# sen-ye/dmvae

Hardware: AMD Instinct MI355X
Metric: images/sec DMVAE train step @256x256 (higher is better)
Workload: dtype bf16

## Files before the change

### dmvae_amd/_lib.py

```python
from __future__ import annotations

import ctypes
import os
from ctypes import POINTER, Structure, c_char_p, c_double, c_float, c_int, c_int32, c_longlong, c_size_t, c_uint, c_ulonglong, c_void_p

_HERE = os.path.dirname(os.path.abspath(__file__))
LIB_PATH = os.environ.get("DMVAE_LIB") or os.path.join(_HERE, "libdmvae_hip.so")


class ConvDesc(Structure):
    _fields_ = [("n", c_int32), ("h", c_int32), ("w", c_int32), ("cin", c_int32), ("cout", c_int32),
                ("ks", c_int32), ("upsample", c_int32), ("act", c_int32), ("out_f32", c_int32), ("stride", c_int32), ("transposed", c_int32),
                ("w_layout", c_int32)]


class PackEntry(Structure):
    _fields_ = [("src", c_void_p), ("dst", c_void_p), ("dst2", c_void_p),
                ("cout", c_int32), ("cin", c_int32), ("T", c_int32), ("rows_pad", c_int32), ("cols_pad", c_int32), ("mode", c_int32), ("subpixel", c_int32),
                ("reserved", c_int32), ("start", c_ulonglong), ("count", c_ulonglong)]


class WtEntry(Structure):
    _fields_ = [("src", c_void_p), ("dst", c_void_p), ("N", c_int32), ("K", c_int32), ("start", c_uint), ("tiles_x", c_uint)]


class OdeTerms(Structure):
    _fields_ = [("k", c_void_p * 7), ("c", c_float * 7), ("nk", c_int32), ("k_bf16", c_int32)]


class ModelTerms(Structure):
    _fields_ = [("kind", c_int32), ("c0", c_float), ("dv", c_float), ("nsig", c_float)]


IMAGE_RECORD_WORDS = 12
IMAGE_OUT_U8_NHWC, IMAGE_OUT_F32_NCHW = 0, 1


ABI_VERSION = 9

SIGNATURES = {
    "dmvae_last_error": (c_char_p, []),
    "dmvae_abi_version": (c_int, []),
    "dmvae_rms_modulate_fwd_f32": (c_int, [c_void_p] * 6 + [c_size_t, c_int, c_int, c_int, c_float, c_void_p]),
    "dmvae_rms_modulate_bwd_f32": (c_int, [c_void_p] * 8 + [c_size_t, c_int, c_int, c_int, c_void_p]),
    "dmvae_layernorm_bwd_full_f32": (c_int, [c_void_p] * 5 + [c_size_t, c_int, c_float, c_void_p]),
    "dmvae_bcast_rows_f32": (c_int, [c_int] + [c_void_p] * 4 + [c_size_t, c_int, c_int, c_int, c_void_p]),
    "dmvae_colsum_groups_f32": (c_int, [c_void_p, c_void_p, c_int, c_int, c_int, c_int, c_void_p]),
    "dmvae_swiglu_fwd_f32": (c_int, [c_void_p, c_void_p, c_size_t, c_int, c_void_p]),
    "dmvae_swiglu_bwd_f32": (c_int, [c_void_p, c_void_p, c_void_p, c_size_t, c_int, c_void_p]),
    "dmvae_qknorm_rope_fwd_f32": (c_int, [c_void_p] * 9 + [c_int] * 5 + [c_float, c_void_p]),
    "dmvae_qknorm_rope_bwd_f32": (c_int, [c_void_p] * 12 + [c_int] * 5 + [c_void_p]),
    "dmvae_reparam_kl_workspace": (c_size_t, [c_size_t, c_int]),
    "dmvae_reparam_kl_fwd": (c_int, [c_void_p] * 5 + [c_size_t, c_size_t, c_int, c_int, c_void_p]),
    "dmvae_reparam_kl_bwd": (c_int, [c_void_p] * 4 + [c_float, c_void_p, c_size_t, c_int, c_int, c_void_p]),
    "dmvae_conv2d_nhwc_fwd": (c_int, [c_void_p, c_void_p, c_void_p, c_void_p, c_void_p, POINTER(ConvDesc), c_void_p]),
    "dmvae_conv2d_nhwc_fwd_gnstats_workspace": (c_size_t, [POINTER(ConvDesc), c_int]),
    "dmvae_conv2d_nhwc_fwd_gnstats": (c_int, [c_void_p] * 7 + [c_size_t, c_int, c_float, POINTER(ConvDesc), c_void_p]),
    "dmvae_conv2d_nhwc_wgrad_workspace": (c_size_t, [POINTER(ConvDesc)]),
    "dmvae_gemm_nt_batched": (c_int, [c_void_p] * 5 + [c_int] * 4 + [c_longlong] * 3 + [c_int, c_int, c_void_p]),
    "dmvae_gemm_tn_batched_workspace": (c_size_t, [c_int, c_int, c_int, c_int]),
    "dmvae_gemm_tn_batched": (c_int, [c_void_p] * 4 + [c_size_t] + [c_int] * 4 + [c_longlong] * 3 + [c_float, c_int, c_void_p]),
    "dmvae_set_dynamic": (c_int, [c_int]),
    "dmvae_linear_rows_supported": (c_int, [c_int, c_int, c_int]),
    "dmvae_linear_rows_bf16": (c_int, [c_void_p] * 4 + [c_int] * 10 + [c_void_p]),
    "dmvae_linear_rows_wgrad": (c_int, [c_void_p] * 4 + [c_int] * 6 + [c_void_p]),
    "dmvae_linear_bf16": (c_int, [c_void_p] * 4 + [c_int] * 10 + [c_void_p]),
    "dmvae_linear_bf16_swiglu_pre": (c_int, [c_void_p] * 5 + [c_int] * 9 + [c_void_p]),
    "dmvae_linear_bf16_sk_supported": (c_int, [c_int] * 5),
    "dmvae_linear_bf16_sk_workspace": (c_size_t, [c_int] * 5),
    "dmvae_linear_bf16_sk": (c_int, [c_void_p] * 5 + [c_size_t] + [c_int] * 11 + [c_void_p]),
    "dmvae_linear_bf16_batched_supported": (c_int, [c_int] * 4),
    "dmvae_linear_bf16_batched": (c_int, [c_void_p] * 3 + [c_int] * 7 + [c_longlong] * 3 + [c_int, c_void_p]),
    "dmvae_linear_bf16_plan": (c_int, [c_int, c_int, c_int, POINTER(c_int), POINTER(c_int)]),
    "dmvae_linear_weight_t_kmajor": (c_int, [c_void_p, c_void_p, c_int, c_int, c_void_p]),
    "dmvae_pack_entry_bytes": (c_size_t, []),
    "dmvae_pack_weights_batched": (c_int, [c_void_p, c_int, c_ulonglong, c_int, c_void_p]),
    "dmvae_softmax_rows_fwd": (c_int, [c_void_p, c_void_p, c_int, c_int, c_float, c_void_p]),
    "dmvae_softmax_rows_bwd": (c_int, [c_void_p, c_void_p, c_void_p, c_int, c_int, c_float, c_void_p]),
    "dmvae_transpose_bf16": (c_int, [c_void_p, c_void_p, c_int, c_int, c_int, c_void_p]),
    "dmvae_pack_conv_weight": (c_int, [c_void_p, c_void_p] + [c_int] * 6 + [c_void_p]),
    "dmvae_pack_conv_weight_v2": (c_int, [c_void_p, c_void_p, c_void_p] + [c_int] * 6 + [c_void_p]),
    "dmvae_conv_halo_applies": (c_int, [POINTER(ConvDesc)]),
    "dmvae_conv_kmajor_applies": (c_int, [POINTER(ConvDesc)]),
    "dmvae_subpixel_weight": (c_int, [c_void_p, c_void_p, c_int, c_int, c_void_p]),
    "dmvae_subpixel_weight_fold": (c_int, [c_void_p, c_void_p, c_int, c_int, c_int, c_void_p]),
    "dmvae_colsum_bf16": (c_int, [c_void_p, c_void_p, c_void_p, c_size_t, c_size_t, c_int, c_int, c_void_p]),
    "dmvae_conv_out_wgrad_workspace": (c_size_t, [c_int, c_int, c_int, c_int, c_int]),
    "dmvae_conv_out_wgrad": (c_int, [c_void_p, c_void_p, c_void_p, c_void_p, c_size_t, c_int, c_int, c_int, c_int, c_int, c_int, c_void_p]),
    "dmvae_sumpool2x2_nhwc": (c_int, [c_void_p, c_void_p, c_int, c_int, c_int, c_int, c_void_p]),
    "dmvae_maxpool2x2_nhwc": (c_int, [c_void_p, c_void_p, c_int, c_int, c_int, c_int, c_void_p]),
    "dmvae_maxpool2x2_relu_bwd_nhwc": (c_int, [c_void_p, c_void_p, c_void_p, c_void_p, c_int, c_int, c_int, c_int, c_void_p]),
    "dmvae_relu_bwd": (c_int, [c_void_p, c_void_p, c_void_p, c_size_t, c_void_p]),
    "dmvae_leaky_relu_bwd": (c_int, [c_void_p, c_void_p, c_void_p, c_size_t, c_float, c_void_p]),
    "dmvae_sde_euler_step": (c_int, [c_void_p, c_void_p, c_int, c_void_p, c_void_p, c_void_p, c_size_t] + [c_float] * 6 + [c_void_p]),
    "dmvae_image_to_u8": (c_int, [c_void_p, c_void_p, c_size_t, c_int, c_int, c_int, c_void_p]),
    "dmvae_ode_rk_combine": (c_int, [c_void_p, POINTER(OdeTerms), c_void_p, c_size_t, c_int, c_void_p]),
    "dmvae_ode_error_ratio_workspace": (c_size_t, [c_size_t]),
    "dmvae_ode_error_ratio": (c_int, [c_void_p, c_void_p, POINTER(OdeTerms), c_float, c_float, c_int, c_void_p, c_void_p, c_void_p, c_size_t, c_void_p]),
    "dmvae_ode_dense_output": (c_int, [c_void_p] * 5 + [c_int, c_float, c_float, c_void_p, c_size_t, c_void_p]),
    "dmvae_ode_hutchinson_pack": (c_int, [c_void_p, c_int, c_void_p, c_void_p, c_void_p, c_void_p, c_int, c_size_t, c_void_p]),
    "dmvae_cfg_combine": (c_int, [c_void_p, c_int, c_void_p, c_int, c_int, c_size_t, c_int, c_float, c_void_p, c_float, c_void_p]),
    "dmvae_sde_heun_perturb": (c_int, [c_void_p, c_void_p, c_void_p, c_size_t, c_float, c_float, c_void_p]),
    "dmvae_sde_heun_predict": (c_int, [c_void_p, c_void_p, c_int, c_void_p, c_void_p, c_size_t] + [c_float] * 4 + [c_void_p]),
    "dmvae_sde_heun_correct": (c_int, [c_void_p, c_void_p, c_void_p, c_void_p, c_int, c_void_p, c_size_t] + [c_float] * 4 + [c_void_p]),
    "dmvae_sde_last_step": (c_int, [c_void_p, c_void_p, c_int, c_void_p, c_size_t, c_int] + [c_float] * 5 + [c_void_p]),
    "dmvae_sde_euler_step_m": (c_int, [c_void_p, c_void_p, c_int, POINTER(ModelTerms), c_void_p, c_void_p, c_void_p, c_size_t] + [c_float] * 6 + [c_void_p]),
    "dmvae_sde_heun_predict_m": (c_int, [c_void_p, c_void_p, c_int, POINTER(ModelTerms), c_void_p, c_void_p, c_size_t] + [c_float] * 4 + [c_void_p]),
    "dmvae_sde_heun_correct_m": (c_int, [c_void_p, c_void_p, c_void_p, c_void_p, c_int, POINTER(ModelTerms), c_void_p, c_size_t] + [c_float] * 4 + [c_void_p]),
    "dmvae_sde_last_step_m": (c_int, [c_void_p, c_void_p, c_int, POINTER(ModelTerms), c_void_p, c_size_t, c_int] + [c_float] * 3 + [c_void_p]),
    "dmvae_model_velocity": (c_int, [c_void_p, c_void_p, c_int, POINTER(ModelTerms), c_void_p, c_size_t, c_void_p]),
    "dmvae_autoguidance_combine": (c_int, [c_void_p, c_int, c_void_p, c_int, c_int, c_void_p, c_int, c_size_t, c_int, c_float, c_void_p, c_float, c_float, c_void_p]),
    "dmvae_batchnorm_running_update": (c_int, [c_void_p, c_void_p, c_void_p, c_int, c_float, c_float, c_float, c_void_p]),
    "dmvae_diffaug_fwd": (c_int, [c_void_p] * 4 + [c_int] * 9 + [c_void_p]),
    "dmvae_diffaug_bwd": (c_int, [c_void_p] * 4 + [c_int] * 9 + [c_void_p]),
    "dmvae_im2col_nhwc_taps": (c_int, [c_void_p, c_void_p] + [c_int] * 8 + [c_void_p]),
    "dmvae_im2col_nhwc_sub": (c_int, [c_void_p, c_void_p] + [c_int] * 9 + [c_void_p]),
    "dmvae_col2im_nhwc": (c_int, [c_void_p, c_void_p] + [c_int] * 8 + [c_void_p]),
    "dmvae_nchw_f32_to_nhwc_bf16": (c_int, [c_void_p, c_void_p, c_int, c_int, c_int, c_int, c_void_p]),
    "dmvae_nhwc_to_nchw_f32": (c_int, [c_void_p, c_void_p, c_int, c_int, c_int, c_int, c_int, c_void_p]),
    "dmvae_silu_fwd": (c_int, [c_void_p, c_void_p, c_size_t, c_void_p]),
    "dmvae_silu_bwd": (c_int, [c_void_p, c_void_p, c_void_p, c_size_t, c_void_p]),
    "dmvae_layernorm_f32_bf16": (c_int, [c_void_p, c_void_p, c_void_p, c_void_p, c_int, c_int, c_float, c_void_p]),
    "dmvae_scale_residual_layernorm": (c_int, [c_void_p] * 6 + [c_int, c_int, c_float, c_void_p]),
    "dmvae_scale_residual_f32": (c_int, [c_void_p, c_void_p, c_void_p, c_size_t, c_int, c_void_p]),
    "dmvae_softmax_rows_bf16": (c_int, [c_void_p, c_void_p, c_size_t, c_int, c_float, c_void_p]),
    "dmvae_attention_qknorm_rope_bf16": (c_int, [c_void_p] * 6 + [c_int] * 4 + [c_float, c_float, c_void_p]),
    "dmvae_attention_qkv_lse_bf16": (c_int, [c_void_p] * 3 + [c_int] * 4 + [c_float, c_void_p]),
    "dmvae_attention_qkv_stream_bf16": (c_int, [c_void_p] * 3 + [c_int] * 4 + [c_float, c_void_p]),
    "dmvae_attention_heads_lse_bf16": (c_int, [c_void_p] * 5 + [c_int] * 5 + [c_float, c_void_p]),
    "dmvae_attention_heads_stream_bf16": (c_int, [c_void_p] * 5 + [c_int] * 5 + [c_float, c_void_p]),
    "dmvae_attention_wide_stream_bf16": (c_int, [c_void_p] * 5 + [c_int] * 3 + [c_float, c_void_p]),
    "dmvae_attention_wide_bwd_stream_bf16": (c_int, [c_void_p] * 10 + [c_int] * 3 + [c_float, c_void_p]),
    "dmvae_attention_bwd_heads_stream_bf16": (c_int, [c_void_p] * 10 + [c_int] * 5 + [c_float, c_void_p]),
    "dmvae_attention_bwd_qkv_lse_bf16": (c_int, [c_void_p] * 5 + [c_int] * 4 + [c_float, c_void_p]),
    "dmvae_attention_bwd_qkv_stream_bf16": (c_int, [c_void_p] * 6 + [c_int] * 4 + [c_float, c_void_p]),
    "dmvae_attention_bwd_heads_lse_bf16": (c_int, [c_void_p] * 9 + [c_int] * 5 + [c_float, c_void_p]),
    "dmvae_vit_bwd_workspace": (c_size_t, [c_int]),
    "dmvae_layernorm_bwd_f32": (c_int, [c_void_p] * 7 + [c_size_t, c_int, c_int, c_float, c_int, c_void_p]),
    "dmvae_layerscale_bwd": (c_int, [c_void_p] * 6 + [c_size_t, c_int, c_int, c_int, c_void_p]),
    "dmvae_gelu_fwd": (c_int, [c_void_p, c_void_p, c_size_t, c_void_p]),
    "dmvae_gelu_bwd": (c_int, [c_void_p, c_void_p, c_void_p, c_size_t, c_void_p]),
    "dmvae_rmsnorm_modulate_bf16": (c_int, [c_void_p] * 4 + [c_int] * 6 + [c_float, c_void_p]),
    "dmvae_gated_residual_rmsnorm_modulate": (c_int, [c_void_p] * 3 + [c_int] * 2 + [c_void_p] * 3 + [c_int] * 6 + [c_float, c_void_p]),
    "dmvae_gated_residual_out": (c_int, [c_void_p] * 4 + [c_int] * 2 + [c_void_p] * 3 + [c_int] * 6 + [c_float, c_void_p]),
    "dmvae_qknorm_rope_bf16": (c_int, [c_void_p] * 8 + [c_int] * 5 + [c_float, c_void_p]),
    "dmvae_swiglu_bf16": (c_int, [c_void_p, c_void_p, c_size_t, c_int, c_void_p]),
    "dmvae_dit_bwd_workspace": (c_size_t, [c_int, c_int]),
    "dmvae_gated_residual_bwd": (c_int, [c_void_p] * 5 + [c_int] * 5 + [c_void_p]),
    "dmvae_swiglu_bwd": (c_int, [c_void_p, c_void_p, c_void_p, c_size_t, c_int, c_void_p]),
    "dmvae_rmsnorm_modulate_bwd": (c_int, [c_void_p] * 8 + [c_size_t] + [c_int] * 6 + [c_float, c_int, c_void_p]),
    "dmvae_qknorm_rope_bwd": (c_int, [c_void_p] * 12 + [c_size_t] + [c_int] * 5 + [c_float, c_int, c_void_p]),
    "dmvae_qknorm_rope_bwd_nblk": (c_int, [c_int] * 5),
    "dmvae_qknorm_rope_bwd_partial": (c_int, [c_void_p] * 10 + [c_size_t] + [c_int] * 5 + [c_float, c_void_p]),
    "dmvae_qknorm_rope_bwd_dx": (c_int, [c_void_p] * 9 + [c_int] * 5 + [c_float, c_void_p]),
    "dmvae_layernorm_modulate_bf16": (c_int, [c_void_p] * 3 + [c_int] * 6 + [c_float, c_void_p]),
    "dmvae_gated_residual_layernorm_modulate": (c_int, [c_void_p] * 4 + [c_int] * 2 + [c_void_p] * 2 + [c_int] * 6 + [c_float, c_void_p]),
    "dmvae_layernorm_modulate_bwd_workspace": (c_size_t, [c_int, c_int, c_int]),
    "dmvae_layernorm_modulate_bwd": (c_int, [c_void_p] * 6 + [c_size_t] + [c_int] * 6 + [c_float, c_void_p]),
    "dmvae_head_split_bf16": (c_int, [c_void_p] * 8 + [c_int] * 7 + [c_float, c_void_p]),
    "dmvae_head_split_bwd_nblk": (c_int, [c_int] * 3),
    "dmvae_head_split_bwd": (c_int, [c_void_p] * 12 + [c_size_t] + [c_int] * 7 + [c_float, c_int, c_void_p]),
    "dmvae_gelu_tanh_fwd": (c_int, [c_void_p, c_void_p, c_size_t, c_void_p]),
    "dmvae_gelu_tanh_bwd": (c_int, [c_void_p, c_void_p, c_void_p, c_size_t, c_void_p]),
    "dmvae_dit_stack_bps": (c_int, [c_int]),
    "dmvae_dit_stack_part_bytes": (c_size_t, [c_int, c_int, c_int]),
    "dmvae_dit_stack_workspace": (c_size_t, [c_int, c_int, c_int, c_int]),
    "dmvae_dit_boundary_bwd": (c_int, [c_void_p] * 4 + [c_int, c_int, c_float, c_void_p, c_void_p, c_void_p, c_int, c_int, c_void_p, c_void_p, c_void_p, c_int, c_int, c_int, c_void_p]),
    "dmvae_dit_boundary_bwd_dx": (c_int, [c_void_p] * 4 + [c_int, c_int, c_float, c_void_p, c_void_p, c_int, c_int, c_void_p, c_void_p, c_int, c_int, c_int, c_void_p]),
    "dmvae_dit_stack_finalize": (c_int, [c_void_p, c_void_p, c_void_p, c_size_t, c_void_p] + [c_int] * 5 + [c_void_p]),
    "dmvae_colsum2_batched": (c_int, [c_void_p] * 3 + [c_int] * 4 + [c_void_p]),
    "dmvae_linear_rows_batched_bf16": (c_int, [c_void_p, c_longlong, c_void_p, c_void_p, c_void_p, c_longlong] + [c_int] * 11 + [c_void_p]),
    "dmvae_linear_rows_wgrad_batched": (c_int, [c_void_p, c_longlong, c_void_p, c_int, c_void_p, c_void_p, c_void_p, c_void_p] + [c_int] * 6 + [c_void_p]),
    "dmvae_wt_entry_bytes": (c_size_t, []),
    "dmvae_linear_weight_t_kmajor_batched": (c_int, [c_void_p, c_int, c_uint, c_void_p]),
    "dmvae_linear_wgrad_grouped_entry_bytes": (c_size_t, []),
    "dmvae_linear_wgrad_grouped_bias_entry_bytes": (c_size_t, []),
    "dmvae_linear_wgrad_grouped_supported": (c_int, [c_int] * 3),
    "dmvae_linear_wgrad_grouped_bias_parts": (c_int, [c_int]),
    "dmvae_linear_wgrad_grouped_fill": (c_int, [c_void_p] * 7 + [c_int] * 3 + [POINTER(c_uint), POINTER(c_uint)]),
    "dmvae_linear_wgrad_grouped": (c_int, [c_void_p, c_int, c_uint, c_int, c_void_p, c_int, c_uint, c_void_p]),
    "dmvae_linear_wgrad_grouped_chunk_bytes": (c_size_t, []),
    "dmvae_linear_wgrad_grouped_plan": (c_int, [c_void_p, c_int, c_void_p, c_int, POINTER(c_int), POINTER(c_uint), POINTER(c_uint)]),
    "dmvae_linear_wgrad_grouped_xcd": (c_int, [c_void_p, c_void_p, POINTER(c_uint), c_uint, c_int, c_void_p, c_int, c_uint, c_void_p]),
    "dmvae_gated_residual_f32": (c_int, [c_void_p, c_void_p, c_void_p, c_size_t, c_int, c_int, c_int, c_int, c_void_p]),
    "dmvae_loss_workspace": (c_size_t, []),
    "dmvae_l1_mse": (c_int, [c_void_p] * 5 + [c_size_t, c_size_t, c_float, c_float, c_void_p]),
    "dmvae_lpips_diff": (c_int, [c_void_p] * 6 + [c_size_t, c_int, c_int, c_int, c_float, c_int, c_void_p]),
    "dmvae_lpips_diff_pool": (c_int, [c_void_p] * 8 + [c_size_t, c_int, c_int, c_int, c_int, c_float, c_int, c_void_p]),
    "dmvae_dmd_pre": (c_int, [c_void_p] * 4 + [c_int, c_int, c_void_p]),
    "dmvae_dmd_post": (c_int, [c_void_p] * 10 + [c_size_t, c_int, c_int, c_float, c_int, c_void_p]),
    "dmvae_kl_mmd_workspace": (c_size_t, [c_int, c_int, c_int]),
    "dmvae_kl_mmd": (c_int, [c_void_p] * 6 + [c_size_t, c_int, c_int, c_int, c_int, c_float, c_float, c_void_p]),
    "dmvae_grad_norm": (c_int, [c_void_p, c_void_p, c_void_p, c_size_t, c_size_t, c_float, c_int, c_void_p]),
    "dmvae_adamw_ema_step": (c_int, [c_void_p] * 6 + [c_size_t] + [c_float] * 5 + [c_int, c_float, c_void_p]),
    "dmvae_adamw_ema_step_shadow": (c_int, [c_void_p] * 7 + [c_size_t] + [c_float] * 5 + [c_int, c_float, c_void_p]),
    "dmvae_mt_chunk_elems": (c_size_t, []),
    "dmvae_mt_grad_norm_workspace": (c_size_t, [c_size_t]),
    "dmvae_mt_grad_norm": (c_int, [c_void_p, c_size_t, c_void_p, c_size_t, c_void_p, c_void_p, c_size_t, c_float, c_void_p]),
    "dmvae_mt_scale_grads": (c_int, [c_void_p, c_size_t, c_void_p, c_size_t, c_void_p, c_void_p]),
    "dmvae_mt_adamw_ema_step": (c_int, [c_void_p, c_size_t, c_void_p, c_size_t, c_void_p] + [c_float] * 5 + [c_int, c_float, c_void_p]),
    "dmvae_mt_ema": (c_int, [c_void_p, c_size_t, c_void_p, c_size_t, c_float, c_void_p]),
    "dmvae_groupnorm_workspace": (c_size_t, [c_int, c_int, c_int, c_int]),
    "dmvae_groupnorm_stats": (c_int, [c_void_p, c_void_p, c_void_p, c_size_t, c_int, c_int, c_int, c_int, c_float, c_void_p]),
    "dmvae_groupnorm_apply": (c_int, [c_void_p, c_void_p, c_void_p, c_void_p, c_void_p, c_int, c_int, c_int, c_int, c_int, c_void_p]),
    "dmvae_groupnorm_bwd": (c_int, [c_void_p] * 10 + [c_size_t, c_int, c_int, c_int, c_int, c_int, c_int, c_void_p]),
    "dmvae_groupnorm_bwd_colsum": (c_int, [c_void_p] * 11 + [c_size_t] + [c_int] * 7 + [c_void_p]),
    "dmvae_groupnorm_bwd_reduce": (c_int, [c_void_p] * 9 + [c_size_t, c_int, c_int, c_int, c_int, c_int, c_int, c_void_p]),
    "dmvae_groupnorm_bwd_apply": (c_int, [c_void_p] * 8 + [c_int, c_int, c_int, c_int, c_int, c_float, c_void_p]),
    "dmvae_groupnorm_short_supported": (c_int, [c_int] * 5),
    "dmvae_groupnorm_apply_short": (c_int, [c_void_p] * 8 + [c_int] * 6 + [c_void_p]),
    "dmvae_groupnorm_bwd_short_workspace": (c_size_t, [c_int] * 5),
    "dmvae_groupnorm_bwd_short": (c_int, [c_void_p] * 12 + [c_size_t] + [c_int] * 8 + [c_void_p]),
    "dmvae_conv_k4c1_supported": (c_int, [c_int] * 4),
    "dmvae_conv_k4c1_wgrad_workspace": (c_size_t, [c_int]),
    "dmvae_conv_k4c1_fwd": (c_int, [c_void_p] * 4 + [c_int] * 4 + [c_void_p]),
    "dmvae_conv_k4c1_dgrad": (c_int, [c_void_p] * 3 + [c_int] * 4 + [c_void_p]),
    "dmvae_conv_k4c1_wgrad": (c_int, [c_void_p] * 5 + [c_size_t] + [c_int] * 4 + [c_void_p]),
    "dmvae_conv_in3_supported": (c_int, [c_int] * 4),
    "dmvae_conv_in3_workspace": (c_size_t, [c_int] * 3),
    "dmvae_conv_in3": (c_int, [c_void_p, c_void_p, c_int] + [c_void_p] * 6 + [c_size_t] + [c_int] * 5 + [c_void_p]),
    "dmvae_conv_to_image_supported": (c_int, [c_int] * 5),
    "dmvae_conv_to_image": (c_int, [c_void_p] * 5 + [c_int] * 5 + [c_void_p]),
    "dmvae_norm_conv_out_fwd_supported": (c_int, [c_int] * 6),
    "dmvae_norm_conv_out_fwd": (c_int, [c_void_p] * 8 + [c_int] * 6 + [c_void_p]),
    "dmvae_norm_conv_out_bwd_supported": (c_int, [c_int] * 6),
    "dmvae_norm_conv_out_bwd_workspace": (c_size_t, [c_int] * 5),
    "dmvae_norm_conv_out_bwd": (c_int, [c_void_p] * 10 + [c_size_t] + [c_int] * 7 + [c_void_p]),
    "dmvae_conv2d_nhwc_wgrad": (c_int, [c_void_p, c_void_p, c_void_p, c_void_p, c_void_p, c_size_t, POINTER(ConvDesc), c_int, c_void_p]),
    "dmvae_split3_bf16": (c_int, [c_void_p, c_void_p, c_size_t, c_int, c_size_t, c_size_t, c_size_t, c_size_t, c_int, c_void_p]),
    "dmvae_groupnorm_stats_f32": (c_int, [c_void_p, c_void_p, c_int, c_int, c_int, c_int, c_float, c_void_p]),
    "dmvae_groupnorm_apply_f32": (c_int, [c_void_p] * 5 + [c_int] * 5 + [c_void_p]),
    "dmvae_groupnorm_f32_workspace": (c_size_t, [c_int, c_int, c_int]),
    "dmvae_groupnorm_bwd_f32": (c_int, [c_void_p] * 10 + [c_size_t] + [c_int] * 6 + [c_float, c_void_p]),
    "dmvae_eltwise_f32": (c_int, [c_int] + [c_void_p] * 4 + [c_size_t, c_int, c_int, c_float, c_void_p]),
    "dmvae_softmax_rows_fwd_f32": (c_int, [c_void_p, c_void_p, c_int, c_int, c_float, c_void_p]),
    "dmvae_softmax_rows_bwd_f32": (c_int, [c_void_p, c_void_p, c_void_p, c_int, c_int, c_float, c_void_p]),
    "dmvae_pool2x2_f32": (c_int, [c_int] + [c_void_p] * 4 + [c_int] * 4 + [c_void_p]),
    "dmvae_nchw_f32_to_nhwc_f32": (c_int, [c_void_p, c_void_p, c_int, c_int, c_int, c_int, c_void_p]),
    "dmvae_lpips_diff_f32": (c_int, [c_void_p] * 6 + [c_size_t, c_int, c_int, c_int, c_float, c_int, c_void_p]),
    "dmvae_layernorm_f32": (c_int, [c_void_p] * 4 + [c_int, c_int, c_float, c_void_p]),
    "dmvae_conv_tokens_pack": (c_int, [c_void_p] * 4 + [c_int, c_int, c_void_p]),
    "dmvae_conv_tokens_fwd": (c_int, [c_void_p] * 4 + [c_int] * 4 + [c_void_p]),
    "dmvae_conv_tokens_dgrad": (c_int, [c_void_p] * 4 + [c_int] * 4 + [c_void_p]),
    "dmvae_conv_tokens_wgrad_workspace": (c_size_t, [c_int] * 4),
    "dmvae_conv_tokens_wgrad": (c_int, [c_void_p] * 5 + [c_size_t] + [c_int] * 4 + [c_void_p]),
    "dmvae_conv_tokens_fwd_bnact": (c_int, [c_void_p] * 7 + [c_float, c_void_p, c_int, c_int, c_int, c_int, c_void_p]),
    "dmvae_dino_bnact_bwd": (c_int, [c_void_p] * 4 + [c_float, c_void_p, c_size_t, c_int, c_void_p]),
    "dmvae_dino_tap": (c_int, [c_void_p, c_void_p, c_int, c_int, c_int, c_void_p]),
    "dmvae_dino_untap": (c_int, [c_void_p, c_void_p, c_int, c_int, c_int, c_void_p]),
    "dmvae_dino_tail_fwd": (c_int, [c_void_p] * 5 + [c_size_t, c_int, c_void_p]),
    "dmvae_dino_tail_bwd_workspace": (c_size_t, [c_size_t, c_int]),
    "dmvae_dino_tail_bwd": (c_int, [c_void_p] * 8 + [c_size_t, c_size_t, c_int, c_void_p]),
    "dmvae_layerscale_bwd_dx": (c_int, [c_void_p, c_void_p, c_void_p, c_size_t, c_int, c_void_p]),
    "dmvae_fid_accumulate": (c_int, [c_void_p, c_int, c_size_t, c_int, c_size_t, c_void_p, c_void_p, c_void_p]),
    "dmvae_fid_resize_u8": (c_int, [c_void_p, c_int, c_size_t, c_int, c_int, c_int, c_void_p, c_void_p]),
    "dmvae_lanczos_kmax": (c_int, [c_int, c_int]),
    "dmvae_lanczos_table": (c_int, [c_int] * 5 + [c_void_p] * 3),
    "dmvae_image_preprocess": (c_int, [c_void_p, c_void_p, c_void_p, c_int, c_int, c_void_p, c_int, c_void_p]),
    "dmvae_ssim_workspace": (c_size_t, [c_size_t, c_int, c_int, c_int]),
    "dmvae_ssim": (c_int, [c_void_p, c_void_p, c_int, c_size_t, c_int, c_int, c_int, c_int, c_double, c_void_p, c_void_p, c_void_p]),
    "dmvae_resize_tf1_bilinear": (c_int, [c_void_p, c_size_t, c_int, c_int, c_int, c_int, c_int, c_void_p, c_void_p]),
    "dmvae_inception_score_workspace": (c_size_t, [c_size_t, c_int, c_size_t]),
    "dmvae_inception_score": (c_int, [c_void_p, c_int, c_size_t, c_int, c_size_t, c_void_p, c_size_t, c_void_p, c_void_p, c_void_p]),
}

_lib = None


class DmvaeHipError(RuntimeError):
    pass


def lib() -> ctypes.CDLL:
    global _lib
    if _lib is None:
        if not os.path.exists(LIB_PATH):
            raise DmvaeHipError(
                f"{LIB_PATH} not found: build it with `python -c 'import __graft_entry__ as g; g.build()'` "
                "or `make -C dmvae_amd/csrc` (there is no CPU fallback)")
        l = ctypes.CDLL(LIB_PATH)
        l.dmvae_abi_version.restype, l.dmvae_abi_version.argtypes = c_int, []
        if l.dmvae_abi_version() != ABI_VERSION:
            raise DmvaeHipError(f"{LIB_PATH}: ABI version {l.dmvae_abi_version()}, this package binds version {ABI_VERSION}; rebuild the library")
        for name, (res, args) in SIGNATURES.items():
            fn = getattr(l, name, None)
            if fn is None:
                raise DmvaeHipError(f"{LIB_PATH} does not export {name} (declared in include/dmvae_hip.h); rebuild the library")
            fn.restype, fn.argtypes = res, args
        _lib = l
# ... 8 lines not shown
```

### dmvae_amd/csrc/common.h

```cpp
#pragma once
#include <hip/hip_runtime.h>
#include <stdint.h>

typedef __bf16 bf16;
typedef __attribute__((ext_vector_type(8))) __bf16 bf16x8;
typedef __attribute__((ext_vector_type(4))) __bf16 bf16x4;
typedef __attribute__((ext_vector_type(2))) __bf16 bf16x2;
typedef __attribute__((ext_vector_type(4))) short s16x4;
typedef __attribute__((ext_vector_type(16))) float f32x16;
typedef __attribute__((ext_vector_type(4))) float f32x4;
typedef __attribute__((ext_vector_type(2))) float f32x2;

#define GPTR(p) ((const __attribute__((address_space(1))) void*)(p))
#define LPTR(p) ((__attribute__((address_space(3))) void*)(p))

static __device__ uint4 dmvae_zero_page[4];

void dmvae_set_error(const char* fmt, ...);
#define DMVAE_CHECK_ARG(cond, ...) do { if (!(cond)) { dmvae_set_error(__VA_ARGS__); return -22; } } while (0)
#define DMVAE_CHECK_LAUNCH() do { hipError_t e_ = hipGetLastError(); if (e_ != hipSuccess) { dmvae_set_error("%s:%d launch failed: %s", __FILE__, __LINE__, hipGetErrorString(e_)); return -5; } } while (0)

static inline int grid_for(size_t n, int block, int cap) {
  size_t g = (n + block - 1) / block;
  return (int)(g > (size_t)cap ? cap : (g < 1 ? 1 : g));
}

struct dmvae_lds_seen { unsigned long long devs; };
int dmvae_lds_optin(dmvae_lds_seen* seen, const void* kernel, int bytes, const char* file, int line);
#define DMVAE_LDS_OPTIN(bytes, ...) do { static dmvae_lds_seen seen_; if (dmvae_lds_optin(&seen_, reinterpret_cast<const void*>(__VA_ARGS__), (int)(bytes), __FILE__, __LINE__)) return -5; } while (0)


__device__ __forceinline__ __amdgpu_buffer_rsrc_t dmvae_buffer_rsrc(const void* p, unsigned bytes) {
  return __builtin_amdgcn_make_buffer_rsrc(const_cast<void*>(p), 0, bytes, 0x00020000);
}
constexpr unsigned SENT = 0x80000000u;

__device__ __forceinline__ int swz64(int row) { return (0 - (row >> 2)) & 3; }

template <int N>
__device__ __forceinline__ void wait_vmcnt() {
  static_assert(N >= 0 && N < 64, "vmcnt is a 6-bit field on gfx9");
  __builtin_amdgcn_s_waitcnt((N & 15) | 0x0F70 | ((N >> 4) << 14));
  asm volatile("" ::: "memory");
}

template <int OFF>
__device__ __forceinline__ s16x4 tr_read_uncounted(unsigned lds_addr) {
  s16x4 r;
  asm volatile("ds_read_b64_tr_b16 %0, %1 offset:%2" : "=v"(r) : "v"(lds_addr), "n"(OFF));
  return r;
}
__device__ __forceinline__ s16x4 tr_read_ordered(const char* p) {
  return __builtin_amdgcn_ds_read_tr16_b64_v4i16((__attribute__((address_space(3))) s16x4*)(p));
}

__device__ __forceinline__ float wave_sum(float v) {
#pragma unroll
  for (int o = 32; o > 0; o >>= 1) v += __shfl_xor(v, o, 64);
  return v;
}
__device__ __forceinline__ float bf2f(bf16 v) { return (float)v; }
__device__ __forceinline__ float sigmoidf_(float x) { return __builtin_amdgcn_rcpf(1.0f + __expf(-x)); }
__device__ __forceinline__ float sigmoid_exact(float x) { return 1.0f / (1.0f + expf(-x)); }

__device__ __forceinline__ float dmvae_gelu_f(float x) {
  const float z = fabsf(x) * 0.70710678118654752f;
  const float t = __builtin_amdgcn_rcpf(__builtin_fmaf(0.3275911f, z, 1.0f));
  float p = __builtin_fmaf(1.061405429f, t, -1.453152027f);
  p = __builtin_fmaf(p, t, 1.421413741f);
  p = __builtin_fmaf(p, t, -0.284496736f);
  p = __builtin_fmaf(p, t, 0.254829592f);
  const float e = p * t * __expf(-z * z);
  return 0.5f * x * (x < 0.f ? e : 2.0f - e);
}

__device__ __forceinline__ unsigned xcd_remap(unsigned flat, unsigned total) {
  const unsigned q = total >> 3, r = total & 7u, x = flat & 7u;
  const unsigned start = x < r ? x * (q + 1) : r * (q + 1) + (x - r) * q;
  return start + (flat >> 3);
}

__device__ __forceinline__ bf16x8 dmvae_ldnt8(const bf16* p) {
  return __builtin_nontemporal_load(reinterpret_cast<const bf16x8*>(p));
}
__device__ __forceinline__ unsigned dmvae_pack_bf16x2(float a, float b) {
  bf16x2 t = {(bf16)a, (bf16)b};
  return *reinterpret_cast<unsigned*>(&t);
}
__device__ __forceinline__ uint4 dmvae_norm_rope8(const uint4 raw, float r, const float* __restrict__ w, const float* __restrict__ cosb,
                                            const float* __restrict__ sinb, int tok, int D, int d0) {
  const bf16x8 x = *reinterpret_cast<const bf16x8*>(&raw);
  const float4 w0 = *reinterpret_cast<const float4*>(w + d0), w1 = *reinterpret_cast<const float4*>(w + d0 + 4);
  const float4 c0 = *reinterpret_cast<const float4*>(cosb + (size_t)tok * D + d0), c1 = *reinterpret_cast<const float4*>(cosb + (size_t)tok * D + d0 + 4);
  const float4 s0 = *reinterpret_cast<const float4*>(sinb + (size_t)tok * D + d0), s1 = *reinterpret_cast<const float4*>(sinb + (size_t)tok * D + d0 + 4);
  const float wv[8] = {w0.x, w0.y, w0.z, w0.w, w1.x, w1.y, w1.z, w1.w};
  const float cv[8] = {c0.x, c0.y, c0.z, c0.w, c1.x, c1.y, c1.z, c1.w};
  const float sv[8] = {s0.x, s0.y, s0.z, s0.w, s1.x, s1.y, s1.z, s1.w};
  float n[8];
#pragma unroll
  for (int e = 0; e < 8; e++) n[e] = (float)(bf16)((float)x[e] * r) * wv[e];
  uint4 o;
  o.x = dmvae_pack_bf16x2(n[0] * cv[0] - n[1] * sv[0], n[1] * cv[1] + n[0] * sv[1]);
  o.y = dmvae_pack_bf16x2(n[2] * cv[2] - n[3] * sv[2], n[3] * cv[3] + n[2] * sv[3]);
  o.z = dmvae_pack_bf16x2(n[4] * cv[4] - n[5] * sv[4], n[5] * cv[5] + n[4] * sv[5]);
  o.w = dmvae_pack_bf16x2(n[6] * cv[6] - n[7] * sv[6], n[7] * cv[7] + n[6] * sv[7]);
  return o;
}
__device__ __forceinline__ float dmvae_sumsq8(const uint4 raw) {
  const bf16x8 x = *reinterpret_cast<const bf16x8*>(&raw);
  float s = 0.f;
#pragma unroll
  for (int e = 0; e < 8; e++) s += (float)x[e] * (float)x[e];
  return s;
}
```

### dmvae_amd/csrc/conv_pp.hip

```cpp
#include "common.h"
#include "dmvae_hip.h"
#include <cstdlib>
#include <atomic>
#include <mutex>
#include <type_traits>
#include <unordered_map>


namespace dmvae_conv_pp {

struct Args {
  const bf16* x;
  const bf16* w;
  const float* bias;
  const bf16* res;
  void* y;
  int N, Hi, Wi, Cin, Ho, Wo, Cout;
  int ks, act, M, ctiles, total;
  int so, pd, sd;
  int Ml;
  unsigned wsRow, wsTap, wsChunk;
  float* gnpart;
  unsigned* sched;
  unsigned long long* dbg;
};

__device__ __forceinline__ int hswz(int row) { return (row >> 1) & 2; }

__device__ __forceinline__ void divmod_small(int m, int d, float inv_d, bool, int& q, int& r) {
  q = (int)((float)m * inv_d);
  r = m - q * d;
  if (r < 0) { q--; r += d; }
  if (r >= d) { q++; r -= d; }
}

template <int TM, int TP, int WM, int WP, int NBUF, bool UPS, bool OUT_F32, bool KO, bool GEN = false, bool SUB = false, bool DYN = false, bool STATS = false,
          bool HALO = false>
__global__ __launch_bounds__(512) void conv_pp_kernel(Args a) {
#if __HIP_DEVICE_COMPILE__
  constexpr int BM = TM / WM / 32, BP = TP / WP / 32;
  constexpr int TILE_A = TM * 64, TILE_B = TP * 64, SLOT = TILE_A + TILE_B;
  constexpr int NPA = TM >= 128 ? TM / 128 : 1, NPB = TP / 128;
  static_assert(TM >= 128 || HALO, "the 64-row tile exists in the halo form only");
  constexpr int NP = NPA + NPB;
  constexpr int PF = NBUF - 1;
  static_assert(WM * WP == 8 && BM * BP == 8, "8 waves x 8 accumulators");
  static_assert(!HALO || (!UPS && !GEN && !SUB && KO && NBUF == 4), "HALO: plain 3x3, chunk-outer K order");
  constexpr int NPH = NPB + 1;
  constexpr int HALO_B = (TP + 16) * 64;
  constexpr int GROUP = 2 * TILE_A + HALO_B;
  constexpr int EPI_OFF = HALO ? GROUP : 2 * SLOT;
  constexpr int EPI_BYTES = 8 * 32 * (((BM >= 4 ? BM / 2 : BM) * 32) * 4 + 16);
  constexpr int DUMP_OFF = GROUP + (GROUP > EPI_BYTES ? GROUP : EPI_BYTES);
  constexpr bool DIRECT = HALO && !OUT_F32;
  constexpr int BM16 = BM * 2, BP16 = BP * 2;
  extern __shared__ __attribute__((aligned(16))) char smem[];

  const int tid = threadIdx.x, lane = tid & 63;
  const int wave = __builtin_amdgcn_readfirstlane(tid >> 6);
  const int grp = wave >> 2;
  const int wm = wave / WP, wp = wave % WP;
  static_assert(!SUB || (!UPS && !GEN && KO), "SUB: its own instantiation, chunk-outer K order");
  const int T = SUB ? 4 : a.ks * a.ks;
  const int TW = SUB ? 16 : T;
  const int nchunk = a.Cin >> 5;
  const int nK = T * nchunk;

  const unsigned wbytes = (unsigned)a.Cout * TW * a.Cin * 2u;
  const unsigned xbytes = (unsigned)a.N * a.Hi * a.Wi * a.Cin * 2u;
  const int SR = GEN ? ((UPS || a.ks == 1) ? 0 : (a.sd == 2 ? 1 : a.pd)) : 1;
  const int sds = GEN && a.sd == 2 ? 1 : 0;
  const unsigned shift = GEN ? ((!UPS && a.ks != 1) ? (unsigned)(SR * a.Wi + SR) * a.Cin * 2u : 0u)
                             : ((!UPS && (SUB || a.ks == 3)) ? (unsigned)(a.Wi + 1) * a.Cin * 2u : 0u);
  const __amdgpu_buffer_rsrc_t rA = dmvae_buffer_rsrc(a.w, wbytes);
  const __amdgpu_buffer_rsrc_t rB =
      dmvae_buffer_rsrc(reinterpret_cast<const char*>(a.x) - shift, xbytes + shift);

  const int dvw = SUB ? a.Wi : a.Wo;
  const int hw = SUB ? a.Hi * a.Wi : a.Ho * a.Wo;
  const float inv_hw = 1.0f / (float)hw, inv_wo = 1.0f / (float)dvw;
  const bool small_m = a.M < (1 << 24);
  int m0 = 0, n0 = 0;
  int par = 0;
  unsigned voffA[NPA];
  unsigned ctrB[NPB], maskB[NPB], selB[NPB];
  unsigned rowo[UPS ? NPB : 1][3], colo[UPS ? NPB : 1][3];
  unsigned ctrH[HALO ? NPH : 1], mskH[HALO ? NPH : 1];
  int it_ky = 0;
  int it = 0, it_tap = 0, it_ch = 0;
  unsigned soffB_tap = 0;
  auto setup = [&](unsigned work) {
    int lane_s = lane;
    if constexpr (DIRECT) asm volatile("" : "+v"(lane_s));
    const unsigned wid = xcd_remap(work, a.total);
    if constexpr (SUB) {
      const unsigned q = wid / a.ctiles;
      n0 = (int)(wid - q * a.ctiles) * TM;
      par = __builtin_amdgcn_readfirstlane((int)(q & 3u));
      m0 = (int)(q >> 2) * TP;
    } else {
      m0 = (int)(wid / a.ctiles) * TP;
      n0 = (int)(wid % a.ctiles) * TM;
    }
    it = it_tap = it_ch = 0;
    it_ky = 0;
#pragma unroll
    for (int p = 0; p < NPA; p++) {
      const int row = (wave * NPA + p) * 16 + (lane_s >> 2);
      int co = n0 + row;
      if constexpr (DIRECT) {
        constexpr int CW_ = TM / WM;
        const int wmr = row / CW_, rr = row % CW_;
        co = n0 + wmr * CW_ + BM16 * (rr & 15) + (rr >> 4);
      }
      const int c = (lane_s & 3) ^ swz64(row);
      voffA[p] = (co < a.Cout && row < TM) ? (unsigned)co * a.wsRow + c * 16u : SENT;
    }
    if constexpr (HALO) {
#pragma unroll
      for (int q = 0; q < NPH; q++) {
        const int i = (q < NPB ? (wave * NPB + q) * 16 : TP) + (lane_s >> 2);
        const int own = min(max(i - 1, 0), TP - 1);
// ... 249 lines not shown
      __builtin_amdgcn_sched_barrier(0);
#pragma unroll
      for (int i = 0; i < BM16; i++)
#pragma unroll
        for (int j = 0; j < BP16; j++) {
          if constexpr (DIRECT) asm volatile("v_mfma_f32_16x16x32_bf16 %0, %1, %2, %0" : "+a"(acc[i][j]) : "v"(bfr[j]), "v"(af[i]));
          else asm volatile("v_mfma_f32_16x16x32_bf16 %0, %1, %2, %0" : "+a"(acc[i][j]) : "v"(af[i]), "v"(bfr[j]));
        }
      __builtin_amdgcn_sched_barrier(0);
      __builtin_amdgcn_s_barrier();
      __builtin_amdgcn_sched_barrier(0);
    };
#pragma unroll 1
    for (int t = 0; t < nK; t += 3) { ktile(K0_{}); ktile(K1_{}); ktile(K2_{}); }
  } else {
#pragma unroll 1
  for (int t = 0; t < nK; t++) {
    const char* sb = smem + slot_rd;
#pragma unroll
    for (int j = 0; j < BP16; j++) bfr[j] = *reinterpret_cast<const bf16x8*>(sb + boff[j]);
#pragma unroll
    for (int i = 0; i < BM16; i++) af[i] = *reinterpret_cast<const bf16x8*>(sb + aoff[i]);
    issue(slot_wr);
    slot_rd = slot_rd + SLOT == NBUF * SLOT ? 0 : slot_rd + SLOT;
    slot_wr = slot_wr + SLOT == NBUF * SLOT ? 0 : slot_wr + SLOT;
    wait_vmcnt<(PF - 1) * NP>();
    __builtin_amdgcn_s_waitcnt(0xC07F);
    asm volatile("" ::: "memory");
    __builtin_amdgcn_sched_barrier(0);
    __builtin_amdgcn_s_barrier();
    __builtin_amdgcn_sched_barrier(0);
#pragma unroll
    for (int i = 0; i < BM16; i++)
#pragma unroll
      for (int j = 0; j < BP16; j++)
        asm volatile("v_mfma_f32_16x16x32_bf16 %0, %1, %2, %0" : "+a"(acc[i][j]) : "v"(af[i]), "v"(bfr[j]));
    __builtin_amdgcn_sched_barrier(0);
    __builtin_amdgcn_s_barrier();
    __builtin_amdgcn_sched_barrier(0);
  }
  }
  stamp(work, 3);
  if (grp == 0) __builtin_amdgcn_s_barrier();
  if constexpr (DYN) next_dyn = __hip_atomic_load(a.sched + 16 + blockIdx.x, __ATOMIC_ACQUIRE, __HIP_MEMORY_SCOPE_WORKGROUP);
  wait_vmcnt<0>();
  asm volatile("s_nop 15\n\ts_nop 15" ::: "memory");

  __builtin_amdgcn_s_barrier();
  stamp(work, 6);
  const unsigned next = DYN ? (unsigned)__builtin_amdgcn_readfirstlane((int)next_dyn) : work + gridDim.x;
  const bool has_next = next < (unsigned)a.total;
  if constexpr (DIRECT) {
    typedef unsigned u32x4 __attribute__((ext_vector_type(4)));
    typedef unsigned u32x2 __attribute__((ext_vector_type(2)));
    constexpr int CL = BM16;
    constexpr int NQD = CL / 4;
    static_assert(CL == 8 || CL == 4, "DIRECT: 8 or 4 couts per lane");
    int lane_o = lane;
    asm volatile("" : "+v"(lane_o));
    const int cc = lane_o & 15, gq = lane_o >> 4;
    const int col = n0c + wm * (TM / WM) + CL * cc;
    const bool c_ok = col < a.Cout;
    const __amdgpu_buffer_rsrc_t rY = dmvae_buffer_rsrc(a.y, (unsigned)a.M * (unsigned)a.Cout * 2u);
    const __amdgpu_buffer_rsrc_t rBias = dmvae_buffer_rsrc(a.bias, a.bias ? (unsigned)a.Cout * 4u : 0u);
    float bsv[CL];
    {
      const unsigned vo = c_ok ? (unsigned)col * 4u : SENT;
#pragma unroll
      for (int h = 0; h < NQD; h++) {
        const u32x4 b4 = __builtin_amdgcn_raw_buffer_load_b128(rBias, vo == SENT ? SENT : vo + 16u * h, 0, 0);
        const f32x4 bf = *reinterpret_cast<const f32x4*>(&b4);
#pragma unroll
        for (int e = 0; e < 4; e++) bsv[4 * h + e] = bf[e];
      }
    }
    if (has_next) {
      stamp(next, 0);
      setup(next);
      stamp(next, 1);
    } else {
      it = (nK + 3) & ~3;
      it_ky = it_ch = 0;
    }
    issue_h(K0_{});
    stamp(work, 7);
    float s1[STATS ? NQD : 1], s2[STATS ? NQD : 1];
    if constexpr (STATS) {
#pragma unroll
      for (int h = 0; h < NQD; h++) { s1[h] = 0.f; s2[h] = 0.f; }
    }
    const unsigned vbase = c_ok ? ((unsigned)(m0c + wp * (TP / WP) + 4 * gq) * (unsigned)a.Cout + (unsigned)col) * 2u : SENT;
    const unsigned rstep = (unsigned)a.Cout * 2u;
    auto body = [&](auto RESc, auto ACTc) __attribute__((always_inline)) {
      constexpr bool RES = decltype(RESc)::value;
      constexpr int ACTC = decltype(ACTc)::value;
      const __amdgpu_buffer_rsrc_t rR = dmvae_buffer_rsrc(a.res, RES ? (unsigned)a.M * (unsigned)a.Cout * 2u : 0u);
      typedef std::conditional_t<CL == 8, u32x4, u32x2> rvec;
      rvec rnx[RES ? 4 : 1];
      auto fetch = [&](int j, int r) {
        if constexpr (RES) {
          if constexpr (CL == 8) rnx[RES ? r : 0] = __builtin_amdgcn_raw_buffer_load_b128(rR, vbase, (unsigned)(j * 16 + r) * rstep, 2);
          else rnx[RES ? r : 0] = __builtin_amdgcn_raw_buffer_load_b64(rR, vbase, (unsigned)(j * 16 + r) * rstep, 2);
        }
      };
#pragma unroll
      for (int r = 0; r < 4; r++) fetch(0, r);
#pragma unroll
      for (int j = 0; j < BP16; j++) {
#pragma unroll
        for (int r = 0; r < 4; r++) {
          float v[CL];
#pragma unroll
          for (int i = 0; i < CL; i++) {
            float x;
            asm volatile("v_accvgpr_read_b32 %0, %1" : "=v"(x) : "a"(acc[i][j][r]));
            v[i] = x + bsv[i];
          }
          const int act = ACTC >= 0 ? ACTC : a.act;
          if constexpr (RES) {
            float rf[CL];
            {
              const rvec rv = rnx[RES ? r : 0];
#pragma unroll
              for (int h = 0; h < CL / 2; h++) {
                const unsigned wd = rv[h];
                const bf16x2 b2 = *reinterpret_cast<const bf16x2*>(&wd);
                rf[2 * h] = (float)b2[0]; rf[2 * h + 1] = (float)b2[1];
              }
            }
            if (j + 1 < BP16) fetch(j + 1, r);
            if (act == 3) {
#pragma unroll
              for (int e = 0; e < CL; e++) v[e] = rf[e] > 0.f ? v[e] : 0.f;
            } else {
#pragma unroll
              for (int e = 0; e < CL; e++) v[e] += rf[e];
            }
          }
          if (act == 1) {
#pragma unroll
            for (int e = 0; e < CL; e++) v[e] = v[e] * sigmoidf_(v[e]);
          } else if (act == 2) {
#pragma unroll
            for (int e = 0; e < CL; e++) v[e] = v[e] > 0.f ? v[e] : 0.f;
          } else if (act == 4) {
#pragma unroll
            for (int e = 0; e < CL; e++) v[e] = v[e] > 0.f ? v[e] : 0.2f * v[e];
          }
          const unsigned so = (unsigned)(j * 16 + r) * rstep;
          unsigned pk[CL / 2];
#pragma unroll
          for (int h = 0; h < CL / 2; h++) pk[h] = dmvae_pack_bf16x2(v[2 * h], v[2 * h + 1]);
          if constexpr (STATS) {
            const bf16x2 one2 = {(bf16)1.0f, (bf16)1.0f};
#pragma unroll
            for (int h = 0; h < CL / 2; h++) {
              const bf16x2 p2 = *reinterpret_cast<const bf16x2*>(&pk[h]);
              s1[STATS ? h >> 1 : 0] = __builtin_amdgcn_fdot2_f32_bf16(p2, one2, s1[STATS ? h >> 1 : 0], false);
              s2[STATS ? h >> 1 : 0] = __builtin_amdgcn_fdot2_f32_bf16(p2, p2, s2[STATS ? h >> 1 : 0], false);
            }
          }
          if constexpr (CL == 8) {
            const u32x4 o = {pk[0], pk[1], pk[2], pk[3]};
            __builtin_amdgcn_raw_buffer_store_b128(o, rY, vbase, so, 2 );
            asm volatile("s_nop 0" :: "v"(o));
          } else {
            const u32x2 o = {pk[0], pk[1]};
            __builtin_amdgcn_raw_buffer_store_b64(o, rY, vbase, so, 2 );
            asm volatile("s_nop 0" :: "v"(o));
          }
        }
      }
    };
    using T_ = std::true_type; using F_ = std::false_type;
    if (a.res) {
      if (a.act == 0) body(T_{}, std::integral_constant<int, 0>{});
      else if (a.act == 3) body(T_{}, std::integral_constant<int, 3>{});
      else body(T_{}, std::integral_constant<int, -1>{});
    } else {
      if (a.act == 0) body(F_{}, std::integral_constant<int, 0>{});
      else if (a.act == 2) body(F_{}, std::integral_constant<int, 2>{});
      else body(F_{}, std::integral_constant<int, -1>{});
    }
    if constexpr (STATS) {
      const size_t trow = (size_t)(m0c / TP) * WP + wp;
#pragma unroll
      for (int h = 0; h < NQD; h++) {
        float t1 = s1[STATS ? h : 0], t2 = s2[STATS ? h : 0];
        t1 += __shfl_xor(t1, 16, 64); t2 += __shfl_xor(t2, 16, 64);
        t1 += __shfl_xor(t1, 32, 64); t2 += __shfl_xor(t2, 32, 64);
        const int cq = col + 4 * h;
        if (gq == 0 && cq < a.Cout) *reinterpret_cast<f32x2*>(a.gnpart + (trow * (a.Cout >> 2) + (cq >> 2)) * 2) = f32x2{t1, t2};
      }
    }
  } else {
    constexpr int EH = BM >= 4 ? BM / 2 : BM;
    constexpr int NH = BM / EH;
    constexpr int CWH = EH * 32;
    constexpr int ROWB = CWH * 4 + 16;
    constexpr int LPR = CWH / 8, RPI = 64 / LPR;
    constexpr int NI = 32 / RPI;
    constexpr unsigned ES = OUT_F32 ? 4u : 2u;
    static_assert(!STATS || !OUT_F32, "STATS: statistics of the bf16 result");
    typedef unsigned u32x4 __attribute__((ext_vector_type(4)));
    char* reg = smem + EPI_OFF + wave * (32 * ROWB);
    int lane_o = lane;
    asm volatile("" : "+v"(lane_o));
    const int cl = lane_o % LPR, rg = lane_o / LPR;
    const unsigned mout = SUB ? 4u * (unsigned)a.M : (unsigned)a.M;
    const __amdgpu_buffer_rsrc_t rY = dmvae_buffer_rsrc(a.y, mout * (unsigned)a.Cout * ES);
    const __amdgpu_buffer_rsrc_t rBias = dmvae_buffer_rsrc(a.bias, a.bias ? (unsigned)a.Cout * 4u : 0u);
    f32x4 bias_lo[NH], bias_hi[NH];
#pragma unroll
    for (int hh = 0; hh < NH; hh++) {
      const int cb = n0c + wm * (TM / WM) + hh * CWH + cl * 8;
      const unsigned vo = cb < a.Cout ? (unsigned)cb * 4u : SENT;
      const u32x4 b0 = __builtin_amdgcn_raw_buffer_load_b128(rBias, vo, 0, 0), b1 = __builtin_amdgcn_raw_buffer_load_b128(rBias, vo + 16u, 0, 0);
      bias_lo[hh] = *reinterpret_cast<const f32x4*>(&b0);
      bias_hi[hh] = *reinterpret_cast<const f32x4*>(&b1);
    }
    if (has_next) {
      stamp(next, 0);
      setup(next);
      stamp(next, 1);
    } else {
      it = HALO ? (nK + 3) & ~3 : nK;
      it_ky = it_ch = 0;
    }
    if constexpr (HALO) issue_h(K0_{}); else issue(0);
    stamp(work, 7);
    float sacc[STATS ? NH : 1][2][2];
    if constexpr (STATS) {
#pragma unroll
      for (int i = 0; i < NH * 4; i++) (&sacc[0][0][0])[i] = 0.f;
    }
    auto body = [&](auto RESc, auto ACTc) __attribute__((always_inline)) {
      constexpr bool RES = decltype(RESc)::value;
      constexpr int ACTC = decltype(ACTc)::value;
      const __amdgpu_buffer_rsrc_t rR = dmvae_buffer_rsrc(a.res, RES ? mout * (unsigned)a.Cout * 2u : 0u);
#pragma unroll
      for (int hh = 0; hh < NH; hh++) {
        if (n0c + wm * (TM / WM) + hh * CWH >= a.Cout) continue;
        const int cb = n0c + wm * (TM / WM) + hh * CWH + cl * 8;
        const bool c_ok = cb < a.Cout;
        const unsigned row_e = (unsigned)(m0c + wp * (TP / WP) + rg) * (unsigned)a.Cout + (unsigned)cb;
        const unsigned ybase = c_ok ? row_e * ES : SENT, rbase = c_ok ? row_e * 2u : SENT;
        const unsigned ystep = (unsigned)(RPI * a.Cout) * ES, rstep = (unsigned)(RPI * a.Cout) * 2u;
        auto sub_off = [&](int j, int it2) -> unsigned {
          const int m = m0c + wp * (TP / WP) + j * 32 + it2 * RPI + rg;
          int n, r, y, x;
          divmod_small(m, hw, inv_hw, small_m, n, r);
          divmod_small(r, dvw, inv_wo, small_m, y, x);
          const unsigned mo = (unsigned)((n * a.Ho + 2 * y + (parc >> 1)) * a.Wo + 2 * x + (parc & 1));
          return (m < a.M && c_ok) ? mo * (unsigned)a.Cout + (unsigned)cb : SENT;
        };
        auto stage = [&](int j) {
#pragma unroll
// ... 57 lines not shown
              for (int e = 0; e < 8; e++) v[e] = v[e] * sigmoidf_(v[e]);
            } else if (act == 2) {
#pragma unroll
              for (int e = 0; e < 8; e++) v[e] = v[e] > 0.f ? v[e] : 0.f;
            } else if (act == 4) {
#pragma unroll
              for (int e = 0; e < 8; e++) v[e] = v[e] > 0.f ? v[e] : 0.2f * v[e];
            }
            unsigned voff = ybase, soff = (unsigned)(j * NI + it2) * ystep;
            if constexpr (SUB) {
              const unsigned eo = sub_off(j, it2);
              voff = eo == SENT ? SENT : eo * ES;
              soff = 0u;
            }
            if constexpr (OUT_F32) {
              const f32x4 o0 = {v[0], v[1], v[2], v[3]}, o1 = {v[4], v[5], v[6], v[7]};
              keep[2 * q] = *reinterpret_cast<const u32x4*>(&o0);
              keep[2 * q + 1] = *reinterpret_cast<const u32x4*>(&o1);
              __builtin_amdgcn_raw_buffer_store_b128(keep[2 * q], rY, voff, soff, 0);
              __builtin_amdgcn_raw_buffer_store_b128(keep[2 * q + 1], rY, voff + 16u, soff, 0);
            } else {
              const u32x4 o = {dmvae_pack_bf16x2(v[0], v[1]), dmvae_pack_bf16x2(v[2], v[3]), dmvae_pack_bf16x2(v[4], v[5]), dmvae_pack_bf16x2(v[6], v[7])};
              if constexpr (STATS) {
                const bf16x2 one2 = {(bf16)1.0f, (bf16)1.0f};
#pragma unroll
                for (int pr = 0; pr < 4; pr++) {
                  const unsigned pw = o[pr];
                  const bf16x2 p2 = *reinterpret_cast<const bf16x2*>(&pw);
                  float& s1 = sacc[STATS ? hh : 0][pr >> 1][0];
                  float& s2 = sacc[STATS ? hh : 0][pr >> 1][1];
                  s1 = __builtin_amdgcn_fdot2_f32_bf16(p2, one2, s1, false);
                  s2 = __builtin_amdgcn_fdot2_f32_bf16(p2, p2, s2, false);
                }
              }
              keep[q] = o;
              __builtin_amdgcn_raw_buffer_store_b128(o, rY, voff, soff, 2);
            }
          }
#pragma unroll
          for (int q = 0; q < (OUT_F32 ? 2 * NQ : NQ); q++) asm volatile("s_nop 0" :: "v"(keep[q]));
          }
        }
      }
    };
    using T_ = std::true_type; using F_ = std::false_type;
    if (a.res) {
      if (a.act == 0) body(T_{}, std::integral_constant<int, 0>{});
      else if (a.act == 3) body(T_{}, std::integral_constant<int, 3>{});
      else body(T_{}, std::integral_constant<int, -1>{});
    } else {
      if (a.act == 0) body(F_{}, std::integral_constant<int, 0>{});
      else if (a.act == 2) body(F_{}, std::integral_constant<int, 2>{});
      else body(F_{}, std::integral_constant<int, -1>{});
    }
    if constexpr (STATS) {
      const size_t trow = (size_t)(SUB ? (m0c / TP) * 4 + parc : m0c / TP) * WP + wp;
#pragma unroll
      for (int hh = 0; hh < NH; hh++)
#pragma unroll
        for (int qd = 0; qd < 2; qd++) {
          float s1 = sacc[STATS ? hh : 0][qd][0], s2 = sacc[STATS ? hh : 0][qd][1];
#pragma unroll
          for (int off = LPR; off < 64; off <<= 1) { s1 += __shfl_xor(s1, off, 64); s2 += __shfl_xor(s2, off, 64); }
          const int cq = n0c + wm * (TM / WM) + hh * CWH + lane_o * 8 + qd * 4;
          if (lane_o < LPR && cq < a.Cout) *reinterpret_cast<f32x2*>(a.gnpart + (trow * (a.Cout >> 2) + (cq >> 2)) * 2) = f32x2{s1, s2};
        }
    }
  }
  if (has_next) { if constexpr (HALO) issue_h(K1_{}); else issue(SLOT); }
  stamp(work, 4);
  wait_vmcnt<HALO ? NPA : NP>();
  stamp(work, 5);
  __builtin_amdgcn_s_barrier();
  if (has_next) { if constexpr (HALO) issue_h(K2_{}); else issue(2 * SLOT); }
  work = next;
  }
  if constexpr (DYN) {
    if (tid == 0 && atomicAdd(a.sched + 8, 1u) == gridDim.x - 1) {
#pragma unroll
      for (int k = 0; k < 9; k++) __hip_atomic_store(a.sched + k, 0u, __ATOMIC_RELAXED, __HIP_MEMORY_SCOPE_AGENT);
    }
  }
#endif
}

constexpr int SCHED_WORDS = 16 + 512, SCHED_SLOTS = 32;
__device__ unsigned g_sched[SCHED_SLOTS * SCHED_WORDS];

static unsigned* sched_for(hipStream_t st) {
  static std::mutex mu;
  static std::unordered_map<unsigned long long, int> slot;
  static std::unordered_map<int, unsigned*> base;
  static std::unordered_map<int, int> used;
  int dev = 0;
  if (hipGetDevice(&dev) != hipSuccess) { (void)hipGetLastError(); return nullptr; }
  std::lock_guard<std::mutex> lk(mu);
  auto b = base.find(dev);
  if (b == base.end()) {
    unsigned* p = nullptr;
    if (hipGetSymbolAddress(reinterpret_cast<void**>(&p), HIP_SYMBOL(g_sched)) != hipSuccess) { (void)hipGetLastError(); return nullptr; }
    b = base.emplace(dev, p).first;
  }
  const unsigned long long key = ((unsigned long long)(unsigned)dev << 56) ^ (unsigned long long)reinterpret_cast<uintptr_t>(st);
  auto it = slot.find(key);
  if (it == slot.end()) {
    int& n = used[dev];
    if (n >= SCHED_SLOTS) return nullptr;
    it = slot.emplace(key, n++).first;
  }
  return b->second + (size_t)it->second * SCHED_WORDS;
}

static std::atomic<int> g_dynamic{-1};
static bool dynamic_on() {
  const int v = g_dynamic.load(std::memory_order_relaxed);
  if (v >= 0) return v != 0;
  static const bool env = [] { const char* e = getenv("DMVAE_PP_DYNAMIC"); return e ? atoi(e) != 0 : false; }();
  return env;
}

template <int TM, int TP, int WM, int WP, int NBUF, bool UPS, bool F32, bool KO, bool GEN = false, bool SUB = false, bool DYN = false, bool STATS = false,
          bool HALO = false>
int launch(Args a, hipStream_t st) {
  a.ctiles = (a.Cout + TM - 1) / TM;
  a.total = ((a.M + TP - 1) / TP) * a.ctiles * (SUB ? 4 : 1);
  constexpr int persist = 256;
  const unsigned grid = (persist > 0 && a.total > persist) ? (unsigned)persist : (unsigned)a.total;
  if constexpr (!DYN && !UPS && KO && !F32) {
    if (dynamic_on() && grid == 256u && (unsigned)a.total > grid) {
      a.sched = sched_for(st);
      if (a.sched) return launch<TM, TP, WM, WP, NBUF, UPS, F32, KO, GEN, SUB, true, STATS, HALO>(a, st);
    }
  }
  constexpr int cwh = (TM / WM / 32 >= 4) ? TM / WM / 2 : TM / WM;
  constexpr int ring = NBUF * (TM + TP) * 64, epi = 2 * (TM + TP) * 64 + 8 * 32 * (cwh * 4 + 16);
  constexpr int group = 2 * TM * 64 + (TP + 16) * 64, epi_h = 8 * 32 * (cwh * 4 + 16);
  constexpr int lds = HALO ? group + (group > epi_h ? group : epi_h) + 1024 : (ring > epi ? ring : epi);
  DMVAE_LDS_OPTIN(lds, conv_pp_kernel<TM, TP, WM, WP, NBUF, UPS, F32, KO, GEN, SUB, DYN, STATS, HALO>);
  hipLaunchKernelGGL((conv_pp_kernel<TM, TP, WM, WP, NBUF, UPS, F32, KO, GEN, SUB, DYN, STATS, HALO>), dim3(grid), dim3(512), lds, st, a);
  DMVAE_CHECK_LAUNCH();
  return 0;
}

static constexpr int halo_mode() { return 3; }
static constexpr bool korder_on() { return true; }
static bool halo_for(int ks, int cout, bool plain, bool ups, bool f32) {
  const int h = halo_mode();
  return plain && !ups && !f32 && ks == 3 && h != 0 && korder_on() && (cout > 128 || (h & 2));
}

template <bool UPS, bool F32>
int pick(const Args& a, hipStream_t st, bool gen) {
  if constexpr (!UPS) {
    if (gen) {
      if (a.Cout <= 128) return launch<128, 512, 2, 4, 4, false, F32, true, true>(a, st);
      return launch<256, 256, 2, 4, 4, false, F32, true, true>(a, st);
    }
  }
  if constexpr (UPS) {
    if (a.Cout <= 128) return launch<128, 512, 2, 4, 4, UPS, F32, false>(a, st);
    return launch<256, 256, 2, 4, 4, UPS, F32, false>(a, st);
  } else {
    if constexpr (!F32) {
      if (halo_for(a.ks, a.Cout, !gen, UPS, F32)) {
        if (a.Cout > 128) return a.gnpart ? launch<256, 256, 2, 4, 4, false, false, true, false, false, false, true, true>(a, st)
                                          : launch<256, 256, 2, 4, 4, false, false, true, false, false, false, false, true>(a, st);
// ... 16 lines not shown

static unsigned long long* g_dbg = nullptr;
extern "C" void dmvae_debug_timing(void* buf) { g_dbg = (unsigned long long*)buf; }

__global__ __launch_bounds__(64) void occupy_kernel(unsigned long long ticks) {
  extern __shared__ char occ[];
  occ[threadIdx.x] = 0;
  const unsigned long long t0 = wall_clock64();
  while (wall_clock64() - t0 < ticks) __builtin_amdgcn_s_sleep(32);
}
extern "C" int dmvae_set_dynamic(int on) {
  dmvae_conv_pp::g_dynamic.store(on < 0 ? -1 : (on != 0), std::memory_order_relaxed);
  return dmvae_conv_pp::dynamic_on() ? 1 : 0;
}

extern "C" int dmvae_debug_occupy(int blocks, int lds_bytes, int microseconds, hipStream_t stream) {
  DMVAE_LDS_OPTIN(160 * 1024, occupy_kernel);
  hipLaunchKernelGGL(occupy_kernel, dim3(blocks), dim3(64), lds_bytes, stream, (unsigned long long)microseconds * 100ull);
  DMVAE_CHECK_LAUNCH();
  return 0;
}

int dmvae_conv_geometry(const dmvae_conv_desc* d, int* ho, int* wo, int* so, int* pd, int* sd, int* fl);

extern "C" int dmvae_conv_halo_applies(const dmvae_conv_desc* d) {
  using namespace dmvae_conv_pp;
  if (!d) return 0;
  int ho, wo, so, pd, sd, fl;
  if (dmvae_conv_geometry(d, &ho, &wo, &so, &pd, &sd, &fl) != 0) return 0;
  const bool plain = !(d->upsample == 2 || d->stride == 2 || d->ks == 4 || d->transposed);
  const long long M = (long long)d->n * ho * wo;
  const long long xbytes = (long long)d->n * d->h * d->w * d->cin * 2;
  const long long wbytes = (long long)d->cout * d->ks * d->ks * d->cin * 2;
  constexpr long long min_m = 16384;
  if (d->cin % 32 != 0 || d->cout < 64 || d->cout % 8 != 0 || M < min_m || xbytes + (1ll << 22) >= (1ll << 31) || wbytes >= (1ll << 31)) return 0;
  if (M >= (1ll << 24) || M * d->cout * (d->out_f32 ? 4 : 2) >= (1ll << 31)) return 0;
  return halo_for(d->ks, d->cout, plain, fl != 0, d->out_f32 != 0) ? 1 : 0;
}

extern "C" int dmvae_conv_kmajor_applies(const dmvae_conv_desc* d) {
  using namespace dmvae_conv_pp;
  if (!d) return 0;
  int ho, wo, so, pd, sd, fl;
  if (dmvae_conv_geometry(d, &ho, &wo, &so, &pd, &sd, &fl) != 0) return 0;
  const bool plain = !(d->upsample == 2 || d->stride == 2 || d->ks == 4 || d->transposed);
  const long long M = (long long)d->n * ho * wo;
  const long long xbytes = (long long)d->n * d->h * d->w * d->cin * 2;
  const long long wbytes = (long long)d->cout * d->ks * d->ks * d->cin * 2;
  constexpr long long min_m = 16384;
  if (d->cin % 32 != 0 || d->cout < 64 || d->cout % 8 != 0 || M < min_m || xbytes + (1ll << 22) >= (1ll << 31) || wbytes >= (1ll << 31)) return 0;
  if (M >= (1ll << 24) || M * d->cout * (d->out_f32 ? 4 : 2) >= (1ll << 31)) return 0;
  return 1;
}

int dmvae_conv_pp_try(const void* x, const void* w, const void* bias, const void* residual, void* y, const dmvae_conv_desc* d,
                      hipStream_t stream, float* gnpart, int gn_groups, int* gn_tp) {
  if (gn_tp) *gn_tp = 0;
  using namespace dmvae_conv_pp;
  int ho, wo, so, pd, sd, fl;
  if (dmvae_conv_geometry(d, &ho, &wo, &so, &pd, &sd, &fl) != 0) return 1;
  const bool plain = !(d->upsample == 2 || d->stride == 2 || d->ks == 4 || d->transposed);
  const bool sub = d->transposed && d->ks == 4 && d->stride == 2;
  const int ups = fl ? 1 : 0;
  const long long M = (long long)d->n * ho * wo;
  const long long xbytes = (long long)d->n * d->h * d->w * d->cin * 2;
  const long long wbytes = (long long)d->cout * d->ks * d->ks * d->cin * 2;
  constexpr long long min_m = 16384;
  if (d->cin % 32 != 0 || d->cout < 64 || d->cout % 8 != 0 || M < min_m || xbytes + (1ll << 22) >= (1ll << 31) || wbytes >= (1ll << 31)) return 1;
  if (M >= (1ll << 24)) return 1;
  if (M * d->cout * (d->out_f32 ? 4 : 2) >= (1ll << 31)) return 1;
  if (d->w_layout != 0 && d->w_layout != 1) {
    dmvae_set_error("conv2d_nhwc_fwd: w_layout %d (0 = tap-major, 1 = K-tile-major where dmvae_conv_kmajor_applies(d) is 1)", d->w_layout);
    return -1;
  }
  Args a;
  a.wsRow = d->w_layout ? 64u : (unsigned)(d->ks * d->ks * d->cin) * 2u;
  a.wsTap = d->w_layout ? (unsigned)d->cout * 64u : (unsigned)d->cin * 2u;
  a.wsChunk = d->w_layout ? (unsigned)(d->ks * d->ks) * (unsigned)d->cout * 64u : 64u;
  a.x = (const bf16*)x; a.w = (const bf16*)w; a.bias = (const float*)bias; a.res = (const bf16*)residual; a.y = y;
  a.N = d->n; a.Hi = d->h; a.Wi = d->w; a.Cin = d->cin; a.Cout = d->cout;
  a.Ho = ho; a.Wo = wo; a.so = so; a.pd = pd; a.sd = sd;
  a.ks = d->ks; a.act = d->act; a.M = (int)M; a.ctiles = 0; a.dbg = g_dbg;
  a.Ml = d->n * d->h * d->w;
  a.gnpart = nullptr;
  if (gnpart && gn_tp && !d->out_f32 && (plain || sub) && !ups && gn_groups > 0 && d->cout % gn_groups == 0 && (d->cout / gn_groups) % 4 == 0) {
    const int tp = d->cout <= 128 ? 512 : 256;
    const long long per_image = sub ? (long long)d->h * d->w : (long long)ho * wo;
    if (per_image % tp == 0) { a.gnpart = gnpart; *gn_tp = tp; }
  }
  a.sched = nullptr;
  const bool f32 = d->out_f32 != 0;
  if (sub) {
    a.M = a.Ml;
    if (a.gnpart) {
      if (a.Cout <= 128) return launch<128, 512, 2, 4, 4, false, false, true, false, true, false, true>(a, stream);
      return launch<256, 256, 2, 4, 4, false, false, true, false, true, false, true>(a, stream);
    }
    if (a.Cout <= 128) return f32 ? launch<128, 512, 2, 4, 4, false, true, true, false, true>(a, stream) : launch<128, 512, 2, 4, 4, false, false, true, false, true>(a, stream);
    return f32 ? launch<256, 256, 2, 4, 4, false, true, true, false, true>(a, stream) : launch<256, 256, 2, 4, 4, false, false, true, false, true>(a, stream);
  }
  if (ups) return f32 ? pick<true, true>(a, stream, false) : pick<true, false>(a, stream, false);
  return f32 ? pick<false, true>(a, stream, !plain) : pick<false, false>(a, stream, !plain);
}
```

### dmvae_amd/csrc/groupnorm.hip

```cpp
#include "common.h"
#include "dmvae_hip.h"

namespace dmvae_gn {

struct Geom {
  int HW, C, G, cpg, tp_shift, rows, ppc, nchunk;
};

__device__ __forceinline__ void load8(const bf16* p, float (&v)[8]) {
  const bf16x8 t = *reinterpret_cast<const bf16x8*>(p);
#pragma unroll
  for (int e = 0; e < 8; e++) v[e] = (float)t[e];
}
__device__ __forceinline__ bf16x8 ldraw(const bf16* p) {
  return __builtin_nontemporal_load(reinterpret_cast<const bf16x8*>(p));
}
__device__ __forceinline__ void cvt8(const bf16x8& t, float (&v)[8]) {
#pragma unroll
  for (int e = 0; e < 8; e++) v[e] = (float)t[e];
}
__device__ __forceinline__ void store8(bf16* p, const float (&v)[8]) {
  bf16x8 t;
#pragma unroll
  for (int e = 0; e < 8; e++) t[e] = (bf16)v[e];
// ... 88 lines not shown
      v[u] = i < items ? *reinterpret_cast<const f32x2*>(part + ((size_t)(n * tpi * 4 + r) * cq + grp * qpg + q) * 2) : f32x2{0.f, 0.f};
    }
#pragma unroll
    for (int u = 0; u < 8; u++) { s += v[u][0]; ss += v[u][1]; }
  }
#pragma unroll
  for (int o = 32; o > 0; o >>= 1) { s += __shfl_xor(s, o, 64); ss += __shfl_xor(ss, o, 64); }
  if (lane == 0) {
    const double cnt = (double)(C / G) * HW;
    const double mean = s / cnt;
    double var = ss / cnt - mean * mean;
    if (var < 0) var = 0;
    stats[wid * 2] = (float)mean;
    stats[wid * 2 + 1] = (float)(1.0 / sqrt(var + (double)eps));
  }
}

template <int ACT>
__global__ __launch_bounds__(256) void apply_kernel(const bf16* __restrict__ x, const float* __restrict__ stats,
                                                    const float* __restrict__ gamma, const float* __restrict__ beta,
                                                    bf16* __restrict__ y, Geom g) {
  const int tp = 1 << g.tp_shift;
  const int lane_c = threadIdx.x & (tp - 1), prow = threadIdx.x >> g.tp_shift;
  if (lane_c * 8 >= g.C) return;
  const int n = blockIdx.y;
  const int p0 = blockIdx.x * g.ppc, p1 = min(p0 + g.ppc, g.HW);
  float sc[8], sh[8];
#pragma unroll
  for (int e = 0; e < 8; e++) {
    const int c = lane_c * 8 + e;
    const float* st = stats + ((size_t)n * g.G + c / g.cpg) * 2;
    sc[e] = st[1] * gamma[c];
    sh[e] = beta[c] - st[0] * sc[e];
  }
  const size_t base = (size_t)n * g.HW * g.C + lane_c * 8;
  auto row = [&](const bf16x8& r, int p) {
    float v[8];
    cvt8(r, v);
#pragma unroll
    for (int e = 0; e < 8; e++) {
      const float t = v[e] * sc[e] + sh[e];
      v[e] = ACT == 1 ? t * sigmoidf_(t) : (ACT == 2 ? (t > 0.f ? t : 0.2f * t) : t);
    }
    store8(y + base + (size_t)p * g.C, v);
  };
  int p = p0 + prow;
  for (; p + g.rows < p1; p += 2 * g.rows) {
    const bf16x8 r0 = ldraw(x + base + (size_t)p * g.C), r1 = ldraw(x + base + (size_t)(p + g.rows) * g.C);
    row(r0, p); row(r1, p + g.rows);
  }
  if (p < p1) row(ldraw(x + base + (size_t)p * g.C), p);
}

template <int ACT>
__global__ __launch_bounds__(256) void bwd_partial_kernel(const bf16* __restrict__ da, const bf16* __restrict__ x,
                                                          const float* __restrict__ stats, const float* __restrict__ gamma,
                                                          const float* __restrict__ beta, float* __restrict__ part, Geom g) {
  const int tp = 1 << g.tp_shift;
  const int lane_c = threadIdx.x & (tp - 1), prow = threadIdx.x >> g.tp_shift;
  const bool active = lane_c * 8 < g.C;
  const int n = blockIdx.y;
  const int p0 = blockIdx.x * g.ppc, p1 = min(p0 + g.ppc, g.HW);
  float A[8], B[8];
#pragma unroll
  for (int e = 0; e < 8; e++) { A[e] = 0.f; B[e] = 0.f; }
  if (active) {
    float mu[8], rs[8], ga[8], be[8];
#pragma unroll
    for (int e = 0; e < 8; e++) {
      const int c = lane_c * 8 + e;
      const float* st = stats + ((size_t)n * g.G + c / g.cpg) * 2;
      mu[e] = st[0]; rs[e] = st[1]; ga[e] = gamma[c]; be[e] = beta[c];
    }
    const size_t base = (size_t)n * g.HW * g.C + lane_c * 8;
    auto row = [&](const bf16x8& rx, const bf16x8& rd) {
      float v[8], d[8];
      cvt8(rx, v);
      cvt8(rd, d);
#pragma unroll
      for (int e = 0; e < 8; e++) {
        const float xh = (v[e] - mu[e]) * rs[e];
        float dy = d[e];
        if (ACT == 1) {
          const float t = xh * ga[e] + be[e];
          const float sg = sigmoidf_(t);
          dy *= sg * (1.f + t * (1.f - sg));
        } else if (ACT == 2) {
          dy = xh * ga[e] + be[e] > 0.f ? dy : 0.2f * dy;
        }
        A[e] += dy; B[e] += dy * xh;
      }
    };
    int p = p0 + prow;
    for (; p + g.rows < p1; p += 2 * g.rows) {
      const size_t o0 = base + (size_t)p * g.C, o1 = base + (size_t)(p + g.rows) * g.C;
      const bf16x8 x0 = ldraw(x + o0), d0 = ldraw(da + o0), x1 = ldraw(x + o1), d1 = ldraw(da + o1);
      row(x0, d0); row(x1, d1);
    }
    if (p < p1) row(ldraw(x + base + (size_t)p * g.C), ldraw(da + base + (size_t)p * g.C));
  }
  block_reduce_store(A, B, part, g, lane_c, prow, active);
}

__global__ void bwd_final_kernel(const float* __restrict__ part, const float* __restrict__ gamma, float* __restrict__ AB,
                                 float* __restrict__ S, Geom g, int N) {
  const int wid = (blockIdx.x * blockDim.x + threadIdx.x) >> 6, lane = threadIdx.x & 63;
  if (wid >= N * g.G) return;
  const int n = wid / g.G, grp = wid % g.G;
  double s1 = 0.0, s2 = 0.0;
  __shared__ double red[4][16][65];
  double (*rw)[65] = red[threadIdx.x >> 6];
  for (int c0 = 0; c0 < g.cpg; c0 += 8) {
    double a[8], b[8];
#pragma unroll
    for (int u = 0; u < 8; u++) { a[u] = 0.0; b[u] = 0.0; }
    for (int ch = lane; ch < g.nchunk; ch += 64) {
      f32x2 v[8];
#pragma unroll
      for (int u = 0; u < 8; u++)
        v[u] = c0 + u < g.cpg ? *reinterpret_cast<const f32x2*>(part + ((size_t)(n * g.nchunk + ch) * g.C + grp * g.cpg + c0 + u) * 2) : f32x2{0.f, 0.f};
#pragma unroll
      for (int u = 0; u < 8; u++) { a[u] += v[u][0]; b[u] += v[u][1]; }
    }
#pragma unroll
    for (int u = 0; u < 8; u++) { rw[2 * u][lane] = a[u]; rw[2 * u + 1][lane] = b[u]; }
    __builtin_amdgcn_fence(__ATOMIC_RELEASE, "wavefront");
    __builtin_amdgcn_wave_barrier();
    __builtin_amdgcn_fence(__ATOMIC_ACQUIRE, "wavefront");
    const int v = lane & 15, q = lane >> 4;
    double t = 0.0;
#pragma unroll
    for (int i = 0; i < 16; i++) t += rw[v][16 * q + i];
    t += __shfl_xor(t, 16, 64);
    t += __shfl_xor(t, 32, 64);
    {
      const int u = v >> 1, c = grp * g.cpg + c0 + u;
      if (lane < 16 && c0 + u < g.cpg) AB[((size_t)n * g.C + c) * 2 + (v & 1)] = (float)t;
    }
#pragma unroll
    for (int u = 0; u < 8; u++) {
      const double au = __shfl(t, 2 * u, 64), bu = __shfl(t, 2 * u + 1, 64);
      if (c0 + u < g.cpg) {
        const int c = grp * g.cpg + c0 + u;
        s1 += (double)gamma[c] * au; s2 += (double)gamma[c] * bu;
      }
    }
    __builtin_amdgcn_fence(__ATOMIC_RELEASE, "wavefront");
    __builtin_amdgcn_wave_barrier();
  }
  if (lane == 0) { S[wid * 2] = (float)s1; S[wid * 2 + 1] = (float)s2; }
}

__global__ void bwd_param_kernel(const float* __restrict__ AB, float* __restrict__ dgamma, float* __restrict__ dbeta, int N, int C,
                                 int accumulate) {
  const int c = blockIdx.x * blockDim.x + threadIdx.x;
  if (c >= C) return;
  double a = 0.0, b = 0.0;
  for (int n = 0; n < N; n++) { a += AB[((size_t)n * C + c) * 2]; b += AB[((size_t)n * C + c) * 2 + 1]; }
  dbeta[c] = (accumulate ? dbeta[c] : 0.f) + (float)a;
  dgamma[c] = (accumulate ? dgamma[c] : 0.f) + (float)b;
}

template <int ACT, bool COLS = false>
__global__ __launch_bounds__(256) void bwd_apply_kernel(const bf16* __restrict__ da, const bf16* __restrict__ x,
                                                        const bf16* __restrict__ dres, const float* __restrict__ stats,
                                                        const float* __restrict__ S, const float* __restrict__ gamma,
                                                        const float* __restrict__ beta, bf16* __restrict__ dx, Geom g, float inv_count,
                                                        float* __restrict__ colpart = nullptr, const float* __restrict__ AB = nullptr,
                                                        float* __restrict__ dgamma = nullptr, float* __restrict__ dbeta = nullptr, int N = 0, int accumulate = 0) {
  if (AB && blockIdx.x == 0 && blockIdx.y == 0) {
    for (int c = threadIdx.x; c < g.C; c += 256) {
      double a = 0.0, b = 0.0;
      int n = 0;
      for (; n + 8 <= N; n += 8) {
        f32x2 v[8];
#pragma unroll
        for (int u = 0; u < 8; u++) v[u] = *reinterpret_cast<const f32x2*>(AB + ((size_t)(n + u) * g.C + c) * 2);
#pragma unroll
        for (int u = 0; u < 8; u++) { a += v[u][0]; b += v[u][1]; }
      }
      for (; n < N; n++) { a += AB[((size_t)n * g.C + c) * 2]; b += AB[((size_t)n * g.C + c) * 2 + 1]; }
      dbeta[c] = (accumulate ? dbeta[c] : 0.f) + (float)a;
      dgamma[c] = (accumulate ? dgamma[c] : 0.f) + (float)b;
    }
  }
  const int tp = 1 << g.tp_shift;
  const int lane_c = threadIdx.x & (tp - 1), prow = threadIdx.x >> g.tp_shift;
  if (!COLS && lane_c * 8 >= g.C) return;
  const bool live = lane_c * 8 < g.C;
  const int n = blockIdx.y;
  const int p0 = blockIdx.x * g.ppc, p1 = live ? min(p0 + g.ppc, g.HW) : p0;
  const float inv_m = inv_count > 0.f ? inv_count : 1.0f / ((float)g.cpg * (float)g.HW);
  float mu[8], rs[8], ga[8], be[8], s1[8], s2[8];
  float cs[COLS ? 8 : 1];
  if constexpr (COLS) {
#pragma unroll
    for (int e = 0; e < 8; e++) cs[e] = 0.f;
  }
#pragma unroll
  for (int e = 0; e < 8; e++) {
    const int c = live ? lane_c * 8 + e : 0;
    const size_t gi = ((size_t)n * g.G + c / g.cpg) * 2;
    mu[e] = stats[gi]; rs[e] = stats[gi + 1]; ga[e] = gamma[c]; be[e] = beta[c];
    s1[e] = S[gi] * inv_m; s2[e] = S[gi + 1] * inv_m;
  }
  const size_t base = (size_t)n * g.HW * g.C + lane_c * 8;
  auto row = [&](const bf16x8& rx, const bf16x8& rd, const bf16x8& ro, int p) {
    float v[8], d[8], o[8];
    cvt8(rx, v);
    cvt8(rd, d);
    if (dres) cvt8(ro, o);
#pragma unroll
    for (int e = 0; e < 8; e++) {
      const float xh = (v[e] - mu[e]) * rs[e];
      float dy = d[e];
      if (ACT == 1) {
        const float t = xh * ga[e] + be[e];
        const float sg = sigmoidf_(t);
        dy *= sg * (1.f + t * (1.f - sg));
      } else if (ACT == 2) {
        dy = xh * ga[e] + be[e] > 0.f ? dy : 0.2f * dy;
      }
      const float r = rs[e] * (dy * ga[e] - s1[e] - xh * s2[e]);
      o[e] = dres ? o[e] + r : r;
      if constexpr (COLS) cs[e] += (float)(bf16)o[e];
    }
    store8(dx + base + (size_t)p * g.C, o);
  };
  int p = p0 + prow;
  for (; p + g.rows < p1; p += 2 * g.rows) {
    const size_t o0 = base + (size_t)p * g.C, o1 = base + (size_t)(p + g.rows) * g.C;
    const bf16x8 x0 = ldraw(x + o0), d0 = ldraw(da + o0), x1 = ldraw(x + o1), d1 = ldraw(da + o1);
    bf16x8 q0 = x0, q1 = x1;
// ... 153 lines not shown
    }
    __builtin_amdgcn_fence(__ATOMIC_RELEASE, "wavefront");
    __builtin_amdgcn_wave_barrier();
  }
  if constexpr (!APPLY) {
    __syncthreads();
    float* red = reinterpret_cast<float*>(smem);
#pragma unroll
    for (int e = 0; e < 8; e++) { red[threadIdx.x * 16 + e] = A[e >> 1][e & 1]; red[threadIdx.x * 16 + 8 + e] = B[e >> 1][e & 1]; }
    __syncthreads();
    if (threadIdx.x < 128) {
      const int c = threadIdx.x, lc = c >> 3, e = c & 7;
      float a = 0.f, b = 0.f;
      for (int r = 0; r < 16; r++) { const float* qq = red + ((r * 16 + lc) * 16); a += qq[e]; b += qq[8 + e]; }
      float* o = part + ((size_t)(n * g.nchunk + blockIdx.x) * C + c) * 2;
      o[0] = a; o[1] = b;
    }
  }
}

static int make_geom(Geom& g, int N, int HW, int C, int G) {
  if (C <= 0 || C % 8 != 0 || C > 512 || G <= 0 || C % G != 0 || HW <= 0 || N <= 0) return -1;
  g.HW = HW; g.C = C; g.G = G; g.cpg = C / G;
  int tp = 1, sh = 0;
  while (tp < C / 8) { tp <<= 1; sh++; }
  g.tp_shift = sh; g.rows = 256 / tp;
  int nchunk = (2048 + N - 1) / N;
  const int maxc = (HW + g.rows * 4 - 1) / (g.rows * 4);
  if (nchunk > maxc) nchunk = maxc;
  if (nchunk > 2048) nchunk = 2048;
  if (nchunk < 1) nchunk = 1;
  g.ppc = (HW + nchunk - 1) / nchunk;
  g.nchunk = (HW + g.ppc - 1) / g.ppc;
  return 0;
}

}
using namespace dmvae_gn;

extern "C" size_t dmvae_groupnorm_workspace(int n, int hw, int c, int groups) {
  Geom g;
  if (make_geom(g, n, hw, c, groups)) return 0;
  return ((size_t)n * g.nchunk * c * 2 + (size_t)n * c * 2 + (size_t)n * groups * 2) * sizeof(float);
}

extern "C" int dmvae_groupnorm_stats(const void* x, void* stats, void* workspace, size_t workspace_bytes, int n, int hw, int c,
                                     int groups, float eps, hipStream_t stream) {
  Geom g;
  DMVAE_CHECK_ARG(x && stats && workspace, "groupnorm_stats: null pointer");
  DMVAE_CHECK_ARG(make_geom(g, n, hw, c, groups) == 0, "groupnorm_stats: unsupported shape n=%d hw=%d c=%d groups=%d", n, hw, c, groups);
  DMVAE_CHECK_ARG(workspace_bytes >= dmvae_groupnorm_workspace(n, hw, c, groups), "groupnorm_stats: workspace too small");
  hipLaunchKernelGGL(stats_partial_kernel, dim3(g.nchunk, n), dim3(256), 0, stream, (const bf16*)x, (float*)workspace, g);
  DMVAE_CHECK_LAUNCH();
  const int waves = n * groups;
  hipLaunchKernelGGL(stats_final_kernel, dim3((waves + 3) / 4), dim3(256), 0, stream, (const float*)workspace, (float*)stats, g, n, eps);
  DMVAE_CHECK_LAUNCH();
  return 0;
}

int dmvae_gn_stats_from_quads(const float* part, float* stats, int n, int hw, int c, int groups, int tp, float eps, hipStream_t stream) {
  DMVAE_CHECK_ARG(part && stats && groups > 0 && c % groups == 0 && (c / groups) % 4 == 0 && tp > 0 && hw % tp == 0, "gn_stats_from_quads: bad shape");
  const int waves = n * groups;
  hipLaunchKernelGGL(stats_from_quads_kernel, dim3((waves + 3) / 4), dim3(256), 0, stream, part, stats, n, hw, c, groups, tp, eps);
  DMVAE_CHECK_LAUNCH();
  return 0;
}

extern "C" int dmvae_groupnorm_apply(const void* x, const void* stats, const void* gamma, const void* beta, void* y, int n, int hw,
                                     int c, int groups, int act, hipStream_t stream) {
  Geom g;
  DMVAE_CHECK_ARG(x && stats && gamma && beta && y, "groupnorm_apply: null pointer");
  DMVAE_CHECK_ARG(act >= 0 && act <= 2, "groupnorm_apply: act must be 0 (none), 1 (swish) or 2 (LeakyReLU 0.2)");
  DMVAE_CHECK_ARG(make_geom(g, n, hw, c, groups) == 0, "groupnorm_apply: unsupported shape n=%d hw=%d c=%d groups=%d", n, hw, c, groups);
  const dim3 grid(g.nchunk, n);
#define DMVAE_GN_APPLY(A) hipLaunchKernelGGL(apply_kernel<A>, grid, dim3(256), 0, stream, (const bf16*)x, (const float*)stats, \
                                             (const float*)gamma, (const float*)beta, (bf16*)y, g)
  if (act == 1) DMVAE_GN_APPLY(1); else if (act == 2) DMVAE_GN_APPLY(2); else DMVAE_GN_APPLY(0);
#undef DMVAE_GN_APPLY
  DMVAE_CHECK_LAUNCH();
  return 0;
}

static int bwd_reduce_impl(const void* da, const void* x, const void* stats, const void* gamma, const void* beta, void* sums, void* dgamma, void* dbeta,
                           void* workspace, size_t workspace_bytes, int n, int hw, int c, int groups, int act, int accumulate, bool with_param, hipStream_t stream);
extern "C" int dmvae_groupnorm_bwd_reduce(const void* da, const void* x, const void* stats, const void* gamma, const void* beta,
                                          void* sums, void* dgamma, void* dbeta, void* workspace, size_t workspace_bytes, int n, int hw,
                                          int c, int groups, int act, int accumulate, hipStream_t stream) {
  return bwd_reduce_impl(da, x, stats, gamma, beta, sums, dgamma, dbeta, workspace, workspace_bytes, n, hw, c, groups, act, accumulate, true, stream);
}
static int bwd_reduce_impl(const void* da, const void* x, const void* stats, const void* gamma, const void* beta, void* sums, void* dgamma, void* dbeta,
                           void* workspace, size_t workspace_bytes, int n, int hw, int c, int groups, int act, int accumulate, bool with_param, hipStream_t stream) {
  Geom g;
  DMVAE_CHECK_ARG(da && x && stats && gamma && beta && sums && workspace, "groupnorm_bwd_reduce: null pointer");
  DMVAE_CHECK_ARG(act >= 0 && act <= 2, "groupnorm_bwd_reduce: act must be 0, 1 or 2");
  DMVAE_CHECK_ARG(make_geom(g, n, hw, c, groups) == 0, "groupnorm_bwd_reduce: unsupported shape n=%d hw=%d c=%d groups=%d", n, hw, c, groups);
  DMVAE_CHECK_ARG(workspace_bytes >= dmvae_groupnorm_workspace(n, hw, c, groups), "groupnorm_bwd_reduce: workspace too small");
  float* part = (float*)workspace;
  float* AB = part + (size_t)n * g.nchunk * c * 2;
  const dim3 grid(g.nchunk, n);
#define DMVAE_GN_PART(A) hipLaunchKernelGGL(bwd_partial_kernel<A>, grid, dim3(256), 0, stream, (const bf16*)da, (const bf16*)x, \
                                            (const float*)stats, (const float*)gamma, (const float*)beta, part, g)
  if (act == 1) DMVAE_GN_PART(1); else if (act == 2) DMVAE_GN_PART(2); else DMVAE_GN_PART(0);
#undef DMVAE_GN_PART
  DMVAE_CHECK_LAUNCH();
  const int waves = n * groups;
  hipLaunchKernelGGL(bwd_final_kernel, dim3((waves + 3) / 4), dim3(256), 0, stream, part, (const float*)gamma, AB, (float*)sums, g, n);
  DMVAE_CHECK_LAUNCH();
  if (dgamma && dbeta && with_param) {
    hipLaunchKernelGGL(bwd_param_kernel, dim3((c + 255) / 256), dim3(256), 0, stream, AB, (float*)dgamma, (float*)dbeta, n, c, accumulate);
    DMVAE_CHECK_LAUNCH();
  }
  return 0;
}

int dmvae_gn_bwd_reduce_parts(const void* da, const void* x, const void* stats, const void* gamma, const void* beta, void* workspace, size_t workspace_bytes,
                              int n, int hw, int c, int groups, int act, float** AB, float** S, hipStream_t stream) {
  Geom g;
  DMVAE_CHECK_ARG(make_geom(g, n, hw, c, groups) == 0, "groupnorm_bwd_reduce: unsupported shape n=%d hw=%d c=%d groups=%d", n, hw, c, groups);
  *AB = (float*)workspace + (size_t)n * g.nchunk * c * 2;
  *S = *AB + (size_t)n * c * 2;
  return bwd_reduce_impl(da, x, stats, gamma, beta, *S, nullptr, nullptr, workspace, workspace_bytes, n, hw, c, groups, act, 0, false, stream);
}

extern "C" int dmvae_groupnorm_bwd_apply(const void* da, const void* x, const void* dres, const void* stats, const void* sums,
                                         const void* gamma, const void* beta, void* dx, int n, int hw, int c, int groups, int act,
                                         float inv_count, hipStream_t stream) {
  Geom g;
  DMVAE_CHECK_ARG(da && x && stats && sums && gamma && beta && dx, "groupnorm_bwd_apply: null pointer");
  DMVAE_CHECK_ARG(act >= 0 && act <= 2, "groupnorm_bwd_apply: act must be 0, 1 or 2");
  DMVAE_CHECK_ARG(make_geom(g, n, hw, c, groups) == 0, "groupnorm_bwd_apply: unsupported shape n=%d hw=%d c=%d groups=%d", n, hw, c, groups);
  const dim3 grid(g.nchunk, n);
#define DMVAE_GN_BAPPLY(A) hipLaunchKernelGGL(bwd_apply_kernel<A>, grid, dim3(256), 0, stream, (const bf16*)da, (const bf16*)x, (const bf16*)dres, \
                                              (const float*)stats, (const float*)sums, (const float*)gamma, (const float*)beta, (bf16*)dx, g, inv_count)
  if (act == 1) DMVAE_GN_BAPPLY(1); else if (act == 2) DMVAE_GN_BAPPLY(2); else DMVAE_GN_BAPPLY(0);
#undef DMVAE_GN_BAPPLY
  DMVAE_CHECK_LAUNCH();
  return 0;
}

extern "C" int dmvae_groupnorm_bwd(const void* da, const void* x, const void* dres, const void* stats, const void* gamma,
                                   const void* beta, void* dx, void* dgamma, void* dbeta, void* workspace, size_t workspace_bytes,
                                   int n, int hw, int c, int groups, int act, int accumulate, hipStream_t stream) {
  Geom g;
  DMVAE_CHECK_ARG(da && x && stats && gamma && beta && dx && workspace, "groupnorm_bwd: null pointer");
  DMVAE_CHECK_ARG(act >= 0 && act <= 2, "groupnorm_bwd: act must be 0, 1 or 2");
  DMVAE_CHECK_ARG(make_geom(g, n, hw, c, groups) == 0, "groupnorm_bwd: unsupported shape n=%d hw=%d c=%d groups=%d", n, hw, c, groups);
  DMVAE_CHECK_ARG(workspace_bytes >= dmvae_groupnorm_workspace(n, hw, c, groups), "groupnorm_bwd: workspace too small");
  float* AB = (float*)workspace + (size_t)n * g.nchunk * c * 2;
  float* S = AB + (size_t)n * c * 2;
  int rc = bwd_reduce_impl(da, x, stats, gamma, beta, S, dgamma, dbeta, workspace, workspace_bytes, n, hw, c, groups, act, accumulate, false, stream);
  if (rc) return rc;
  const bool par = dgamma && dbeta;
  const dim3 grid(g.nchunk, n);
#define DMVAE_GN_BAPPLYP(A) hipLaunchKernelGGL((bwd_apply_kernel<A, false>), grid, dim3(256), 0, stream, (const bf16*)da, (const bf16*)x, (const bf16*)dres, \
                                               (const float*)stats, (const float*)S, (const float*)gamma, (const float*)beta, (bf16*)dx, g, 0.f, (float*)nullptr, \
                                               par ? (const float*)AB : (const float*)nullptr, (float*)dgamma, (float*)dbeta, n, accumulate)
  if (act == 1) DMVAE_GN_BAPPLYP(1); else if (act == 2) DMVAE_GN_BAPPLYP(2); else DMVAE_GN_BAPPLYP(0);
#undef DMVAE_GN_BAPPLYP
  DMVAE_CHECK_LAUNCH();
  return 0;
}

int dmvae_colsum_final(const float* part, float* out, int nparts, int C, int accumulate, hipStream_t stream);

extern "C" int dmvae_groupnorm_bwd_colsum(const void* da, const void* x, const void* dres, const void* stats, const void* gamma, const void* beta, void* dx,
                                          void* dgamma, void* dbeta, void* colsum, void* workspace, size_t workspace_bytes, int n, int hw, int c, int groups,
                                          int act, int accumulate, int colsum_accumulate, hipStream_t stream) {
  Geom g;
  DMVAE_CHECK_ARG(da && x && stats && gamma && beta && dx && colsum && workspace, "groupnorm_bwd_colsum: null pointer");
  DMVAE_CHECK_ARG(act >= 0 && act <= 2, "groupnorm_bwd_colsum: act must be 0, 1 or 2");
  DMVAE_CHECK_ARG(make_geom(g, n, hw, c, groups) == 0, "groupnorm_bwd_colsum: unsupported shape n=%d hw=%d c=%d groups=%d", n, hw, c, groups);
  DMVAE_CHECK_ARG(workspace_bytes >= dmvae_groupnorm_workspace(n, hw, c, groups), "groupnorm_bwd_colsum: workspace too small");
  float* AB = (float*)workspace + (size_t)n * g.nchunk * c * 2;
  float* S = AB + (size_t)n * c * 2;
  int rc = bwd_reduce_impl(da, x, stats, gamma, beta, S, dgamma, dbeta, workspace, workspace_bytes, n, hw, c, groups, act, accumulate, false, stream);
  if (rc) return rc;
  const bool par = dgamma && dbeta;
  float* colpart = (float*)workspace;
  const dim3 grid(g.nchunk, n);
#define DMVAE_GN_BAPPLYC(A) hipLaunchKernelGGL((bwd_apply_kernel<A, true>), grid, dim3(256), 0, stream, (const bf16*)da, (const bf16*)x, (const bf16*)dres, \
                                               (const float*)stats, (const float*)S, (const float*)gamma, (const float*)beta, (bf16*)dx, g, 0.f, colpart, \
                                               par ? (const float*)AB : (const float*)nullptr, (float*)dgamma, (float*)dbeta, n, accumulate)
  if (act == 1) DMVAE_GN_BAPPLYC(1); else if (act == 2) DMVAE_GN_BAPPLYC(2); else DMVAE_GN_BAPPLYC(0);
#undef DMVAE_GN_BAPPLYC
  DMVAE_CHECK_LAUNCH();
  return dmvae_colsum_final(colpart, (float*)colsum, n * g.nchunk, c, colsum_accumulate, stream);
}

static int convout_geom(Geom& g, int n, int h, int w, int c, int groups) {
  if (n <= 0 || h <= 0 || w <= 0 || c != 128 || groups <= 0 || c % groups != 0 || (c / groups) % 2 != 0 || w % 16 != 0) return -1;
  const long long hw = (long long)h * w;
  if (hw * c * n >= (1ll << 40) || hw >= (1ll << 30)) return -1;
  g.HW = (int)hw; g.C = c; g.G = groups; g.cpg = c / groups; g.tp_shift = 4; g.rows = 16;
  int nchunk = (2048 + n - 1) / n;
  int ppc = (int)((hw + nchunk - 1) / nchunk);
  ppc = (ppc + 15) / 16 * 16;
  if (ppc < 64) ppc = 64;
  g.ppc = ppc; g.nchunk = (int)((hw + ppc - 1) / ppc);
  return 0;
}
extern "C" int dmvae_norm_conv_out_bwd_supported(int n, int h, int w, int c, int groups, int cout) {
  Geom g;
  return (cout == 3 && convout_geom(g, n, h, w, c, groups) == 0) ? 1 : 0;
}
extern "C" size_t dmvae_norm_conv_out_bwd_workspace(int n, int h, int w, int c, int groups) {
  Geom g;
  if (convout_geom(g, n, h, w, c, groups)) return 0;
  return ((size_t)n * g.nchunk * c * 2 + (size_t)n * c * 2 + (size_t)n * groups * 2) * sizeof(float) + (size_t)n * (h + 2) * (w + 2) * 4 * sizeof(bf16);
}
extern "C" int dmvae_norm_conv_out_bwd(const void* dy, const void* w, const void* x, const void* stats, const void* gamma, const void* beta, void* dx, void* dgamma,
                                       void* dbeta, void* workspace, size_t workspace_bytes, int n, int h, int wd, int c, int groups, int cout, int accumulate,
                                       hipStream_t stream) {
  Geom g;
  DMVAE_CHECK_ARG(dy && w && x && stats && gamma && beta && dx && workspace, "norm_conv_out_bwd: null pointer");
  DMVAE_CHECK_ARG(cout == 3 && convout_geom(g, n, h, wd, c, groups) == 0,
                  "norm_conv_out_bwd: unsupported shape n=%d h=%d w=%d c=%d groups=%d cout=%d (c = 128, w %% 16 == 0, cout = 3)", n, h, wd, c, groups, cout);
  DMVAE_CHECK_ARG(workspace_bytes >= dmvae_norm_conv_out_bwd_workspace(n, h, wd, c, groups), "norm_conv_out_bwd: workspace too small");
  DMVAE_CHECK_ARG((dgamma == nullptr) == (dbeta == nullptr), "norm_conv_out_bwd: dgamma and dbeta go together");
  float* part = (float*)workspace;
  float* AB = part + (size_t)n * g.nchunk * c * 2;
  float* S = AB + (size_t)n * c * 2;
  bf16* dyp = (bf16*)(S + (size_t)n * groups * 2);
  const dim3 grid(g.nchunk, n);
  hipLaunchKernelGGL(convout_pad_kernel, dim3((unsigned)(((size_t)n * (h + 2) * (wd + 2) + 255) / 256)), dim3(256), 0, stream, (const float*)dy, dyp, n, h, wd);
  DMVAE_CHECK_LAUNCH();
  hipLaunchKernelGGL(convout_bwd_kernel<false>, grid, dim3(256), 0, stream, (const bf16*)dyp, (const float*)w, (const bf16*)x, (const float*)stats, (const float*)gamma,
                     (const float*)beta, part, (const float*)nullptr, (bf16*)nullptr, g, h, wd, (const float*)nullptr, (float*)nullptr, (float*)nullptr, n, 0);
  DMVAE_CHECK_LAUNCH();
  const int waves = n * groups;
  hipLaunchKernelGGL(bwd_final_kernel, dim3((waves + 3) / 4), dim3(256), 0, stream, part, (const float*)gamma, AB, S, g, n);
  DMVAE_CHECK_LAUNCH();
  hipLaunchKernelGGL(convout_bwd_kernel<true>, grid, dim3(256), 0, stream, (const bf16*)dyp, (const float*)w, (const bf16*)x, (const float*)stats, (const float*)gamma,
                     (const float*)beta, (float*)nullptr, (const float*)S, (bf16*)dx, g, h, wd, dgamma ? (const float*)AB : (const float*)nullptr, (float*)dgamma,
                     (float*)dbeta, n, accumulate);
  DMVAE_CHECK_LAUNCH();
  return 0;
}
```

### dmvae_amd/functional.py

```python
from __future__ import annotations

from typing import Optional
import os

import weakref

import torch

from . import ops, parity
from .ops import bf16, f32

_EPOCH = [0]


def bump_weight_epoch() -> None:
    _EPOCH[0] += 1


def _epoch_of(w) -> int:
    return getattr(w, "_dmvae_epoch", _EPOCH)[0]


def packed(w: torch.Tensor, for_dgrad: bool = False, rows_pad: int = 0, cols_pad: int = 0, frozen: bool = False,
           transposed: bool = False, subpixel: bool = False, kmajor: bool = False) -> torch.Tensor:
# ... 64 lines not shown
            assert p.shape[1] == T and p.is_contiguous()
            p2 = getattr(p, "_dmvae_kmajor", None)
            e = arr[i]
            e.src, e.dst, e.dst2 = ptr, p.data_ptr(), (p2.data_ptr() if p2 is not None else None)
            e.cout, e.cin, e.T, e.rows_pad, e.cols_pad, e.mode, e.subpixel = cout, cin, T, rows_pad, cols_pad, int(for_dgrad), int(subpixel)
            e.start, e.count = start, ((rows_pad + 31) // 32) * ((cols_pad + 31) // 32)
            start += e.count
            taps = max(taps, 9 if subpixel else T)
        assert ctypes.sizeof(_lib.PackEntry) == _lib.lib().dmvae_pack_entry_bytes()
        host = torch.frombuffer(bytearray(bytes(arr)), dtype=torch.uint8)
        dev = next(iter(ents.values()))[0].device
        reg["table"], reg["n"], reg["total"], reg["taps"], reg["dirty"] = host.to(dev), len(ents), start, taps, False
    ops.check(_lib.lib().dmvae_pack_weights_batched(reg["table"].data_ptr(), reg["n"], reg["total"], reg["taps"], ops._stream()), "pack_weights_batched")
    ep = epoch[0]
    for (w, key, p, for_dgrad, subpixel, ptr) in ents.values():
        w._dmvae_packed[key] = ((ptr, _ver(w), ep), p)


DIRECT_GRAD_WRITES = None


def _dst(param):
    if param is None:
        return None
    v = getattr(param, "_dmvae_grad_view", None)
    if v is not None and DIRECT_GRAD_WRITES is not None:
        DIRECT_GRAD_WRITES[id(param)] = DIRECT_GRAD_WRITES.get(id(param), 0) + 1
    return None if v is None else v.view(v.shape)


_GN_CHECK = os.environ.get("DMVAE_GN_STATS_CHECK", "0") != "0"
_GN_GROUPS, _GN_EPS = 32, 1e-6


def _tag_stats(y: torch.Tensor, st: torch.Tensor, groups: int = _GN_GROUPS, eps: float = _GN_EPS) -> torch.Tensor:
    try:
        y._dmvae_gn = (st, _ver(y), y.data_ptr(), groups, eps)
    except AttributeError:
        pass
    return y


def _ver(t: torch.Tensor) -> int:
    return -1 if t.is_inference() else t._version


def _stats_of(x: torch.Tensor, groups: int = _GN_GROUPS, eps: float = _GN_EPS) -> torch.Tensor:
    tag = getattr(x, "_dmvae_gn", None)
    if tag is not None and tag[1] == _ver(x) and tag[2] == x.data_ptr() and tag[0].shape[0] == x.shape[0] and tag[3] == groups and tag[4] == eps:
        if _GN_CHECK:
            ref = ops.groupnorm_stats(x, groups, eps)
            assert torch.allclose(tag[0], ref, rtol=1e-4, atol=1e-6), "stale GroupNorm statistics tag"
        return tag[0]
    return ops.groupnorm_stats(x, groups, eps)


def _gn_swish(x, gw, gb, swish=True):
    st = _stats_of(x)
    return st, ops.groupnorm_apply(x, st, gw, gb, swish)


def _c(t):
    return t if t.is_contiguous() else t.contiguous()


def _lib_mod():
    from . import _lib
    return _lib


SHORTCUT_IN_NORM = True
SHORTCUT_IN_NORM_512 = True


def _shortcut_in_norm(x: torch.Tensor, sw) -> bool:
    if sw is None or not SHORTCUT_IN_NORM or parity.on() or x.dtype != bf16 or sw.dim() != 4 or sw.shape[2] != 1:
        return False
    n, c = x.shape[0], x.shape[-1]
    if c == 512 and not SHORTCUT_IN_NORM_512:
        return False
    return sw.shape[1] == c and ops.groupnorm_short_supported(n, x.numel() // (n * c), c, sw.shape[0])


class ResnetBlockFn(torch.autograd.Function):

    @staticmethod
    def forward(ctx, x, n1w, n1b, c1w, c1b, n2w, n2b, c2w, c2b, sw, sb):
        ctx.short = _shortcut_in_norm(x, sw)
        if ctx.short:
            st1 = _stats_of(x)
            a1, xs = ops.groupnorm_apply_short(x, st1, n1w, n1b, packed(sw), sb)
        else:
            st1, a1 = _gn_swish(x, n1w, n1b)
            xs = x if sw is None else ops.conv2d_nhwc(x, packed(sw), sb, ks=1)
        h1, st2 = ops.conv2d_nhwc_gnstats(a1, packed(c1w), c1b, ks=3)
        a2 = ops.groupnorm_apply(h1, st2, n2w, n2b, True)
        y, sty = ops.conv2d_nhwc_gnstats(a2, packed(c2w), c2b, residual=xs, ks=3)
        ctx.save_for_backward(x, st1, a1, h1, st2, a2, n1w, n1b, c1w, n2w, n2b, c2w, sw)
        ctx.bias_params = (c1b, c2b, sb)
        ctx.want_colsum = bool(getattr(x, "_dmvae_want_colsum", False)) and not parity.on()
        return _tag_stats(y, sty)

    @staticmethod
    def backward(ctx, dy):
        x, st1, a1, h1, st2, a2, n1w, n1b, c1w, n2w, n2b, c2w, sw = ctx.saved_tensors
        dy = _c(dy)
        c1b, c2b, sb = ctx.bias_params
        dc2w, dc2b = ops.conv2d_nhwc_wgrad(dy, a2, 3, dw_out=_dst(c2w), db_out=_dst(c2b))
        da2 = ops.conv2d_nhwc(dy, packed(c2w, True), ks=3)
        dh1, dn2w, dn2b = ops.groupnorm_bwd(da2, h1, st2, n2w, n2b, True, dg_out=_dst(n2w), db_out=_dst(n2b))
        dc1w, dc1b = ops.conv2d_nhwc_wgrad(dh1, a1, 3, dw_out=_dst(c1w), db_out=_dst(c1b))
        da1 = ops.conv2d_nhwc(dh1, packed(c1w, True), ks=3)
        if sw is None:
            dxs, dsw, dsb = dy, None, None
        else:
            dsw, dsb = ops.conv2d_nhwc_wgrad(dy, x, 1, dw_out=_dst(sw), db_out=_dst(sb))
            if ctx.short:
                dx, dn1w, dn1b = ops.groupnorm_bwd_short(da1, x, dy, packed(sw, True), st1, n1w, n1b, True, dg_out=_dst(n1w), db_out=_dst(n1b),
                                                         want_colsum=ctx.want_colsum)
                return dx, dn1w, dn1b, dc1w, dc1b, dn2w, dn2b, dc2w, dc2b, dsw, dsb
            dxs = ops.conv2d_nhwc(dy, packed(sw, True), ks=1)
        dx, dn1w, dn1b = ops.groupnorm_bwd(da1, x, st1, n1w, n1b, True, dres=dxs, dg_out=_dst(n1w), db_out=_dst(n1b), want_colsum=ctx.want_colsum)
        return dx, dn1w, dn1b, dc1w, dc1b, dn2w, dn2b, dc2w, dc2b, dsw, dsb


ATTN_WIDE_STREAM = None


def _attn_wide_stream(s: int, c: int) -> bool:
    if ATTN_WIDE_STREAM is None:
        return s > ops.ATTNBLOCK_COMPOSED_MAX and ops.attention_wide_supported(s, c) and not parity.on()
    return bool(ATTN_WIDE_STREAM)


ATTN_WIDE_BWD_STREAM = None


def _attn_wide_bwd_stream(s: int, c: int, fwd_streamed: bool) -> bool:
    if not fwd_streamed or not ops.attention_wide_supported(s, c) or parity.on():
        return False
    if ATTN_WIDE_BWD_STREAM is None:
        return ATTN_WIDE_STREAM is None
    return bool(ATTN_WIDE_BWD_STREAM)


def _attn_pad(t: torch.Tensor, sp: int) -> torch.Tensor:
    n, s, c = t.shape
    if s == sp:
        return t
    out = t.new_zeros(n, sp, c)
    out[:, :s] = t
    return out


def _attn_probs(q: torch.Tensor, k: torch.Tensor, scale: float, s: int) -> torch.Tensor:
    sc = ops.gemm_nt(q, k, out_f32=True)
    if q.shape[1] != s:
        sc[:, :, s:] = float("-inf")
    return ops.softmax_rows(sc, scale)


class AttnBlockFn(torch.autograd.Function):

    @staticmethod
    def forward(ctx, x, nw, nb, qw, qb, kw, kb, vw, vb, pw, pb):
        n, h, w, c = x.shape
        s = h * w
        sp = (s + 31) // 32 * 32
        st, hn = _gn_swish(x, nw, nb, swish=False)
        q = ops.conv2d_nhwc(hn, packed(qw), qb, ks=1).view(n, s, c)
        k = ops.conv2d_nhwc(hn, packed(kw), kb, ks=1).view(n, s, c)
        v = ops.conv2d_nhwc(hn, packed(vw), vb, ks=1).view(n, s, c)
        scale = float(c) ** -0.5
        ctx.stream = _attn_wide_stream(s, c)
        ctx.bwd_stream = _attn_wide_bwd_stream(s, c, ctx.stream)
        lse = None
        if ctx.bwd_stream:
            o, lse = ops.attention_wide_stream(q, k, v, scale, need_lse=True)
        elif ctx.stream:
            o = ops.attention_wide_stream(q, k, v, scale)
        else:
            p = _attn_probs(_attn_pad(q, sp), _attn_pad(k, sp), scale, s)
            o = ops.gemm_nt(p, ops.transpose_last2(_attn_pad(v, sp)))
            if sp != s:
                o = o[:, :s].contiguous()
        y, sty = ops.conv2d_nhwc_gnstats(o.view(n, h, w, c), packed(pw), pb, residual=x, ks=1)
        if ctx.bwd_stream:
            ctx.save_for_backward(x, st, hn, q, k, v, o, lse, nw, nb, qw, kw, vw, pw)
        elif ctx.stream:
            ctx.save_for_backward(x, st, hn, q, k, v, o, nw, nb, qw, kw, vw, pw)
        else:
            ctx.save_for_backward(x, st, hn, q, k, v, p, o, nw, nb, qw, kw, vw, pw)
        ctx.bias_params = (qb, kb, vb, pb)
        ctx.scale = scale
        return _tag_stats(y, sty)

    @staticmethod
    def backward(ctx, dy):
        if ctx.bwd_stream:
            x, st, hn, q, k, v, o, lse, nw, nb, qw, kw, vw, pw = ctx.saved_tensors
        elif ctx.stream:
            x, st, hn, q, k, v, o, nw, nb, qw, kw, vw, pw = ctx.saved_tensors
        else:
            x, st, hn, q, k, v, p, o, nw, nb, qw, kw, vw, pw = ctx.saved_tensors
        n, h, w, c = x.shape
# ... 1272 lines not shown
```

### dmvae_amd/ops.py

```python
from __future__ import annotations

import ctypes
import os
from typing import Optional, Sequence, Tuple

import torch

from . import _lib, parity
from ._lib import ConvDesc, check

bf16 = torch.bfloat16
f32 = torch.float32

ACT_NONE, ACT_SILU, ACT_RELU, ACT_RELU_GATE, ACT_LEAKY, ACT_GELU = 0, 1, 2, 3, 4, 5
ACT_SWIGLU = 6


def _stream() -> int:
    return torch.cuda.current_stream().cuda_stream


def _req(t: torch.Tensor, dtype, name: str) -> torch.Tensor:
    if not t.is_cuda:
        raise _lib.DmvaeHipError(f"{name}: expected a GPU tensor; dmvae_amd has no CPU path")
# ... 443 lines not shown
    if parity.on():
        return parity.softmax_rows(s, scale)
    s = _req(s, f32, "S")
    p = torch.empty(s.shape, dtype=bf16, device=s.device)
    check(_lib.lib().dmvae_softmax_rows_fwd(s.data_ptr(), p.data_ptr(), s.numel() // s.shape[-1], s.shape[-1], float(scale), _stream()), "softmax_rows_fwd")
    return p


def softmax_rows_bwd(dp: torch.Tensor, p: torch.Tensor, scale: float) -> torch.Tensor:
    if p.dtype == f32 and parity.on():
        return parity.softmax_rows_bwd(dp, p, scale)
    dp = _req(dp, f32, "dP")
    p = _req(p, bf16, "P")
    ds = torch.empty_like(p)
    check(_lib.lib().dmvae_softmax_rows_bwd(dp.data_ptr(), p.data_ptr(), ds.data_ptr(), p.numel() // p.shape[-1], p.shape[-1], float(scale), _stream()),
          "softmax_rows_bwd")
    return ds


def transpose_last2(x: torch.Tensor) -> torch.Tensor:
    if x.dtype == f32 and parity.on():
        return parity.transpose_last2(x)
    x = _req(x, bf16, "x")
    assert x.dim() == 3
    out = torch.empty(x.shape[0], x.shape[2], x.shape[1], dtype=bf16, device=x.device)
    check(_lib.lib().dmvae_transpose_bf16(x.data_ptr(), out.data_ptr(), x.shape[0], x.shape[1], x.shape[2], _stream()), "transpose_bf16")
    return out


def groupnorm_stats(x: torch.Tensor, groups: int = 32, eps: float = 1e-6) -> torch.Tensor:
    if x.dtype == f32 and parity.on():
        return parity.groupnorm_stats(x, groups, eps)
    x = _req(x, bf16, "x")
    n, c = x.shape[0], x.shape[-1]
    hw = x.numel() // (n * c)
    L = _lib.lib()
    wsb = L.dmvae_groupnorm_workspace(n, hw, c, groups)
    if wsb == 0:
        raise ValueError(f"groupnorm: unsupported shape {tuple(x.shape)} with {groups} groups")
    ws = workspace(wsb, x.device)
    stats = torch.empty(n, groups, 2, dtype=f32, device=x.device)
    check(L.dmvae_groupnorm_stats(x.data_ptr(), stats.data_ptr(), ws.data_ptr(), ws.numel(), n, hw, c, groups, float(eps), _stream()), "groupnorm_stats")
    return stats


def groupnorm_apply(x: torch.Tensor, stats: torch.Tensor, gamma: torch.Tensor, beta: torch.Tensor, swish: bool, groups: int = 32) -> torch.Tensor:
    if x.dtype == f32 and parity.on():
        return parity.groupnorm_apply(x, stats, gamma, beta, int(swish), groups)
    x = _req(x, bf16, "x")
    n, c = x.shape[0], x.shape[-1]
    hw = x.numel() // (n * c)
    y = torch.empty_like(x)
    check(_lib.lib().dmvae_groupnorm_apply(x.data_ptr(), _req(stats, f32, "stats").data_ptr(), _req(gamma, f32, "gamma").data_ptr(),
                                           _req(beta, f32, "beta").data_ptr(), y.data_ptr(), n, hw, c, groups, int(swish), _stream()), "groupnorm_apply")
    return y


def groupnorm_bwd(da: torch.Tensor, x: torch.Tensor, stats: torch.Tensor, gamma: torch.Tensor, beta: torch.Tensor, swish: bool,
                  dres: Optional[torch.Tensor] = None, groups: int = 32, need_param_grads: bool = True,
                  dg_out: Optional[torch.Tensor] = None, db_out: Optional[torch.Tensor] = None, want_colsum: bool = False):
    if x.dtype == f32 and parity.on():
        return parity.groupnorm_bwd(da, x, stats, gamma, beta, int(swish), dres, groups, need_param_grads, dg_out, db_out)
    da = _req(da, bf16, "da")
    x = _req(x, bf16, "x")
    n, c = x.shape[0], x.shape[-1]
    hw = x.numel() // (n * c)
    L = _lib.lib()
    wsb = L.dmvae_groupnorm_workspace(n, hw, c, groups)
    ws = workspace(wsb, x.device)
    dx = torch.empty_like(x)
    dg = (dg_out if dg_out is not None else torch.empty(c, dtype=f32, device=x.device)) if need_param_grads else None
    db = (db_out if db_out is not None else torch.empty(c, dtype=f32, device=x.device)) if need_param_grads else None
    if dres is not None:
        _req(dres, bf16, "dres")
    if want_colsum:
        cs = torch.empty(c, dtype=f32, device=x.device)
        check(L.dmvae_groupnorm_bwd_colsum(da.data_ptr(), x.data_ptr(), _ptr(dres), stats.data_ptr(), gamma.data_ptr(), beta.data_ptr(), dx.data_ptr(),
                                           _ptr(dg), _ptr(db), cs.data_ptr(), ws.data_ptr(), ws.numel(), n, hw, c, groups, int(swish), 0, 0, _stream()),
              "groupnorm_bwd_colsum")
        dx._dmvae_colsum = (cs, dx._version, dx.data_ptr())
        return dx, dg, db
    check(L.dmvae_groupnorm_bwd(da.data_ptr(), x.data_ptr(), _ptr(dres), stats.data_ptr(), gamma.data_ptr(), beta.data_ptr(), dx.data_ptr(),
                                _ptr(dg), _ptr(db), ws.data_ptr(), ws.numel(), n, hw, c, groups, int(swish), 0, _stream()), "groupnorm_bwd")
    return dx, dg, db


def conv_in3_supported(n: int, h: int, w: int, cout: int) -> bool:
    return bool(_lib.lib().dmvae_conv_in3_supported(n, h, w, cout))


def conv_in3(x0: torch.Tensor, x1: Optional[torch.Tensor], w: torch.Tensor, bias: Optional[torch.Tensor], shift: Optional[torch.Tensor] = None,
             scale: Optional[torch.Tensor] = None, act: int = ACT_NONE) -> torch.Tensor:
    x0 = _req(x0, f32, "x0")
    w = _req(w, f32, "weight")
    n0, c, h, wd = x0.shape
    n1 = 0
    if x1 is not None:
        x1 = _req(x1, f32, "x1")
        assert tuple(x1.shape[1:]) == (c, h, wd), (x0.shape, x1.shape)
        n1 = x1.shape[0]
    cout = w.shape[0]
    assert c == 3 and tuple(w.shape) == (cout, 3, 3, 3), (x0.shape, w.shape)
    n = n0 + n1
    L = _lib.lib()
    if not L.dmvae_conv_in3_supported(n, h, wd, cout):
        raise ValueError(f"conv_in3: unsupported shape {n} x {h} x {wd} -> {cout}")
    if bias is not None:
        bias = _req(bias, f32, "bias")
    if shift is not None:
        shift, scale = _req(shift.reshape(-1), f32, "shift"), _req(scale.reshape(-1), f32, "scale")
        assert shift.numel() == 3 and scale.numel() == 3
    ws = workspace(L.dmvae_conv_in3_workspace(n, h, wd), x0.device, slot="conv_in3")
    y = torch.empty(n, h, wd, cout, dtype=bf16, device=x0.device)
    check(L.dmvae_conv_in3(x0.data_ptr(), _ptr(x1), n0, _ptr(shift), _ptr(scale), w.data_ptr(), _ptr(bias), y.data_ptr(), ws.data_ptr(), ws.numel(), n, h, wd,
                           cout, act, _stream()), "conv_in3")
    return y


def conv_k4c1_supported(n: int, h: int, w: int, c: int) -> bool:
    return bool(_lib.lib().dmvae_conv_k4c1_supported(n, h, w, c))


def conv_k4c1_fwd(x: torch.Tensor, w: torch.Tensor, bias: Optional[torch.Tensor]) -> torch.Tensor:
    x = _req(x, bf16, "x"); w = _req(w, f32, "weight")
    n, h, wd, c = x.shape
    assert tuple(w.shape) == (1, c, 4, 4), (x.shape, w.shape)
    out = torch.empty(n, h - 1, wd - 1, 1, dtype=f32, device=x.device)
    check(_lib.lib().dmvae_conv_k4c1_fwd(x.data_ptr(), w.data_ptr(), _ptr(None if bias is None else _req(bias, f32, "bias")), out.data_ptr(), n, h, wd, c, _stream()), "conv_k4c1_fwd")
    return out


def conv_k4c1_dgrad(dy: torch.Tensor, w: torch.Tensor, h: int) -> torch.Tensor:
    dy = _req(dy, f32, "dy"); w = _req(w, f32, "weight")
    n, c = dy.shape[0], w.shape[1]
    assert dy.shape[1] == h - 1 and dy.shape[2] == 30
    dx = torch.empty(n, h, 31, c, dtype=bf16, device=dy.device)
    check(_lib.lib().dmvae_conv_k4c1_dgrad(dy.data_ptr(), w.data_ptr(), dx.data_ptr(), n, h, 31, c, _stream()), "conv_k4c1_dgrad")
    return dx


def conv_k4c1_wgrad(x: torch.Tensor, dy: torch.Tensor, dw: Optional[torch.Tensor] = None, db: Optional[torch.Tensor] = None, need_bias: bool = True):
    x = _req(x, bf16, "x"); dy = _req(dy, f32, "dy")
    n, h, wd, c = x.shape
    L = _lib.lib()
    if dw is None:
        dw = torch.empty(1, c, 4, 4, dtype=f32, device=x.device)
    if db is None and need_bias:
        db = torch.empty(1, dtype=f32, device=x.device)
    assert dw.dtype == f32 and dw.is_contiguous() and dw.numel() == 16 * c and (db is None or (db.dtype == f32 and db.numel() == 1))
    ws = workspace(L.dmvae_conv_k4c1_wgrad_workspace(c), x.device, slot="conv_k4c1")
    check(L.dmvae_conv_k4c1_wgrad(x.data_ptr(), dy.data_ptr(), dw.data_ptr(), _ptr(db), ws.data_ptr(), ws.numel(), n, h, wd, c, _stream()), "conv_k4c1_wgrad")
    return dw, db


def conv_to_image_supported(n: int, h: int, w: int, cin: int, cout: int) -> bool:
    return bool(_lib.lib().dmvae_conv_to_image_supported(n, h, w, cin, cout))


def conv_to_image(x: torch.Tensor, w_packed: torch.Tensor, cout: int, bias: Optional[torch.Tensor] = None, mul: Optional[torch.Tensor] = None) -> torch.Tensor:
    x = _req(x, bf16, "x")
    w_packed = _req(w_packed, bf16, "w_packed")
    n, h, wd, cin = x.shape
    assert tuple(w_packed.shape) == (4, 9, cin), w_packed.shape
    if bias is not None:
        bias = _req(bias, f32, "bias")
    if mul is not None:
# ... 1735 lines not shown
```

### include/dmvae_hip.h

```cpp
#ifndef DMVAE_HIP_H
#define DMVAE_HIP_H

#include <stddef.h>
#include <stdint.h>

#ifdef __cplusplus
extern "C" {
#endif

typedef struct ihipStream_t* dmvae_stream_t;

const char* dmvae_last_error(void);
int dmvae_abi_version(void);


typedef struct dmvae_conv_desc {
  int32_t n, h, w;
  int32_t cin, cout;
  int32_t ks;
  int32_t upsample;
  int32_t act;
  int32_t out_f32;
  int32_t stride;
  int32_t transposed;
  int32_t w_layout;
} dmvae_conv_desc;

int dmvae_conv_halo_applies(const dmvae_conv_desc* d);
int dmvae_conv_kmajor_applies(const dmvae_conv_desc* d);

int dmvae_conv2d_nhwc_fwd(const void* x, const void* w, const void* bias, const void* residual, void* y,
                          const dmvae_conv_desc* d, dmvae_stream_t stream);

size_t dmvae_conv2d_nhwc_fwd_gnstats_workspace(const dmvae_conv_desc* d, int groups);
int dmvae_conv2d_nhwc_fwd_gnstats(const void* x, const void* w, const void* bias, const void* residual, void* y, void* stats, void* workspace,
                                  size_t workspace_bytes, int groups, float eps, const dmvae_conv_desc* d, dmvae_stream_t stream);

size_t dmvae_conv2d_nhwc_wgrad_workspace(const dmvae_conv_desc* d);
int dmvae_conv2d_nhwc_wgrad(const void* dy, const void* a, void* dw, void* dbias, void* workspace,
                            size_t workspace_bytes, const dmvae_conv_desc* d, int accumulate,
                            dmvae_stream_t stream);

size_t dmvae_conv_out_wgrad_workspace(int n, int h, int w, int cin, int cout);
int dmvae_conv_out_wgrad(const void* dy, const void* a, void* dw, void* workspace, size_t workspace_bytes, int n, int h, int w, int cin, int cout,
                         int accumulate, dmvae_stream_t stream);


size_t dmvae_groupnorm_workspace(int n, int hw, int c, int groups);

int dmvae_groupnorm_stats(const void* x, void* stats, void* workspace, size_t workspace_bytes, int n, int hw,
                          int c, int groups, float eps, dmvae_stream_t stream);

int dmvae_groupnorm_apply(const void* x, const void* stats, const void* gamma, const void* beta, void* y,
                          int n, int hw, int c, int groups, int act, dmvae_stream_t stream);

int dmvae_groupnorm_bwd(const void* da, const void* x, const void* dres, const void* stats, const void* gamma,
                        const void* beta, void* dx, void* dgamma, void* dbeta, void* workspace,
                        size_t workspace_bytes, int n, int hw, int c, int groups, int act, int accumulate,
                        dmvae_stream_t stream);
int dmvae_groupnorm_bwd_colsum(const void* da, const void* x, const void* dres, const void* stats, const void* gamma, const void* beta, void* dx,
                               void* dgamma, void* dbeta, void* colsum, void* workspace, size_t workspace_bytes, int n, int hw, int c, int groups, int act,
                               int accumulate, int colsum_accumulate, dmvae_stream_t stream);
int dmvae_groupnorm_bwd_reduce(const void* da, const void* x, const void* stats, const void* gamma, const void* beta,
                               void* sums, void* dgamma, void* dbeta, void* workspace, size_t workspace_bytes, int n,
                               int hw, int c, int groups, int act, int accumulate, dmvae_stream_t stream);
int dmvae_groupnorm_bwd_apply(const void* da, const void* x, const void* dres, const void* stats, const void* sums,
                              const void* gamma, const void* beta, void* dx, int n, int hw, int c, int groups, int act,
                              float inv_count, dmvae_stream_t stream);

int dmvae_norm_conv_out_fwd_supported(int n, int h, int w, int c, int groups, int cout);
int dmvae_norm_conv_out_fwd(const void* x, const void* stats, const void* gamma, const void* beta, const void* w, const void* bias, void* a, void* y,
                            int n, int h, int wd, int c, int groups, int cout, dmvae_stream_t stream);
int dmvae_conv_to_image_supported(int n, int h, int w, int cin, int cout);
int dmvae_conv_to_image(const void* x, const void* w, const void* bias, const void* mul, void* y, int n, int h, int wd, int cin, int cout, dmvae_stream_t stream);
int dmvae_norm_conv_out_bwd_supported(int n, int h, int w, int c, int groups, int cout);
size_t dmvae_norm_conv_out_bwd_workspace(int n, int h, int w, int c, int groups);
int dmvae_norm_conv_out_bwd(const void* dy, const void* w, const void* x, const void* stats, const void* gamma, const void* beta, void* dx, void* dgamma,
                            void* dbeta, void* workspace, size_t workspace_bytes, int n, int h, int wd, int c, int groups, int cout, int accumulate,
                            dmvae_stream_t stream);

int dmvae_groupnorm_short_supported(int n, int hw, int c, int cs, int groups);
int dmvae_groupnorm_apply_short(const void* x, const void* stats, const void* gamma, const void* beta, const void* w, const void* bias, void* a, void* xs,
                                int n, int hw, int c, int cs, int groups, int act, dmvae_stream_t stream);
size_t dmvae_groupnorm_bwd_short_workspace(int n, int hw, int c, int cs, int groups);
int dmvae_groupnorm_bwd_short(const void* da, const void* x, const void* dys, const void* wt, const void* stats, const void* gamma, const void* beta,
                              void* dx, void* dgamma, void* dbeta, void* colsum, void* workspace, size_t workspace_bytes, int n, int hw, int c, int cs,
                              int groups, int act, int accumulate, int colsum_accumulate, dmvae_stream_t stream);

int dmvae_conv_in3_supported(int n, int h, int w, int cout);
size_t dmvae_conv_in3_workspace(int n, int h, int w);
int dmvae_conv_in3(const void* x0, const void* x1, int n0, const void* shift, const void* scale, const void* w, const void* bias, void* y,
                   void* workspace, size_t workspace_bytes, int n, int h, int wd, int cout, int act, dmvae_stream_t stream);


int dmvae_gemm_nt_batched(const void* A, const void* B, const void* bias, const void* R, void* C, int M, int N,
                          int K, int batch, long long a_bs, long long b_bs, long long c_bs, int act, int out_f32,
                          dmvae_stream_t stream);

size_t dmvae_gemm_tn_batched_workspace(int M, int N, int K, int batch);
int dmvae_gemm_tn_batched(const void* A, const void* B, void* C, void* workspace, size_t workspace_bytes, int M,
                          int N, int K, int batch, long long a_bs, long long b_bs, long long c_bs, float alpha,
                          int out_f32, dmvae_stream_t stream);

int dmvae_linear_rows_supported(int M, int N, int K);
int dmvae_linear_rows_bf16(const void* x, const void* w, const void* bias, void* y, int M, int N, int K, int ldx, int ldw, int ldy, int act,
                           int bias_bf16, int out_f32, int w_layout, dmvae_stream_t stream);
int dmvae_linear_rows_wgrad(const void* dy, const void* x, void* dw, void* db, int M, int N, int K, int lddy, int ldx, int accumulate, dmvae_stream_t stream);

int dmvae_set_dynamic(int on);

int dmvae_linear_bf16(const void* x, const void* w, const void* bias, void* y, int M, int N, int K, int lda, int ldw, int ldy,
                      int act, int bias_bf16, int out_f32, int w_layout, dmvae_stream_t stream);
int dmvae_linear_bf16_plan(int M, int N, int K, int* tile_cols, int* tile_rows);
int dmvae_linear_bf16_batched_supported(int batch, int M, int N, int K);
int dmvae_linear_bf16_batched(const void* x, const void* w, void* y, int batch, int M, int N, int K, int lda, int ldw, int ldy, long long sx, long long sw,
                              long long sy, int out_f32, dmvae_stream_t stream);
int dmvae_linear_bf16_swiglu_pre(const void* x, const void* w, const void* bias, void* g, void* x12, int M, int N, int K, int lda, int ldw, int ldg,
                                 int ldx12, int bias_bf16, int w_layout, dmvae_stream_t stream);

int dmvae_linear_bf16_sk_supported(int M, int N, int K, int splits, int tile);
size_t dmvae_linear_bf16_sk_workspace(int M, int N, int K, int splits, int tile);
int dmvae_linear_bf16_sk(const void* x, const void* w, const void* bias, void* y, void* workspace, size_t workspace_bytes, int splits, int tile,
                         int M, int N, int K, int lda, int ldw, int ldy, int act, int bias_bf16, int w_layout, dmvae_stream_t stream);
int dmvae_linear_weight_t_kmajor(const void* w, void* out, int N, int K, dmvae_stream_t stream);

int dmvae_softmax_rows_fwd(const void* s, void* p, int rows, int cols, float scale, dmvae_stream_t stream);
int dmvae_softmax_rows_bwd(const void* dp, const void* p, void* ds, int rows, int cols, float scale,
                           dmvae_stream_t stream);
int dmvae_transpose_bf16(const void* src, void* dst, int batch, int rows, int cols, dmvae_stream_t stream);


int dmvae_pack_conv_weight(const void* w, void* out, int cout, int cin, int ks, int rows_pad, int cols_pad,
                           int for_dgrad, dmvae_stream_t stream);
int dmvae_pack_conv_weight_v2(const void* w, void* out, void* out_kmajor, int cout, int cin, int ks, int rows_pad, int cols_pad,
                              int for_dgrad, dmvae_stream_t stream);
typedef struct {
  const float* src; void* dst; void* dst2;
  int32_t cout, cin, T, rows_pad, cols_pad, mode, subpixel, reserved;
  uint64_t start, count;
} dmvae_pack_entry;
size_t dmvae_pack_entry_bytes(void);
int dmvae_pack_weights_batched(const void* table, int n_entries, unsigned long long total, int max_taps, dmvae_stream_t stream);
int dmvae_subpixel_weight(const void* w, void* wd, int cout, int cin, dmvae_stream_t stream);
int dmvae_subpixel_weight_fold(const void* dwd, void* dw, int cout, int cin, int accumulate, dmvae_stream_t stream);
int dmvae_colsum_bf16(const void* x, void* out, void* workspace, size_t workspace_bytes, size_t rows, int cols, int accumulate,
// ... 348 lines not shown
```

Measured before the change: 492.8.

## Fuse GroupNorm backward reductions into the conv dgrad epilogue

Adds a conv dgrad kernel variant whose epilogue, in the halo tile path, reads the GroupNorm input, stats, gamma and beta. It accumulates the per-channel swish-backward partial sums (sum of g and g*xhat) and writes them to a partials buffer. The GroupNorm backward then uses these partials instead of re-reading da and x in a separate reduction pass. The resnet block backward is rewired to use this path when the shape is supported. This saves a full read pass over the activation gradient, at the cost of higher register pressure in the conv epilogue and an extra partials buffer.

```diff
diff --git a/dmvae_amd/_lib.py b/dmvae_amd/_lib.py
--- a/dmvae_amd/_lib.py
+++ b/dmvae_amd/_lib.py
@@ -56,6 +56,9 @@
     "dmvae_conv2d_nhwc_fwd": (c_int, [c_void_p, c_void_p, c_void_p, c_void_p, c_void_p, POINTER(ConvDesc), c_void_p]),
     "dmvae_conv2d_nhwc_fwd_gnstats_workspace": (c_size_t, [POINTER(ConvDesc), c_int]),
     "dmvae_conv2d_nhwc_fwd_gnstats": (c_int, [c_void_p] * 7 + [c_size_t, c_int, c_float, POINTER(ConvDesc), c_void_p]),
+    "dmvae_conv2d_nhwc_gnbwd_supported": (c_int, [POINTER(ConvDesc), c_int]),
+    "dmvae_conv2d_nhwc_gnbwd_workspace": (c_size_t, [POINTER(ConvDesc), c_int]),
+    "dmvae_conv2d_nhwc_gnbwd": (c_int, [c_void_p] * 8 + [c_size_t, c_int, POINTER(ConvDesc), c_void_p]),
     "dmvae_conv2d_nhwc_wgrad_workspace": (c_size_t, [POINTER(ConvDesc)]),
     "dmvae_gemm_nt_batched": (c_int, [c_void_p] * 5 + [c_int] * 4 + [c_longlong] * 3 + [c_int, c_int, c_void_p]),
     "dmvae_gemm_tn_batched_workspace": (c_size_t, [c_int, c_int, c_int, c_int]),
@@ -205,6 +208,8 @@
     "dmvae_groupnorm_apply": (c_int, [c_void_p, c_void_p, c_void_p, c_void_p, c_void_p, c_int, c_int, c_int, c_int, c_int, c_void_p]),
     "dmvae_groupnorm_bwd": (c_int, [c_void_p] * 10 + [c_size_t, c_int, c_int, c_int, c_int, c_int, c_int, c_void_p]),
     "dmvae_groupnorm_bwd_colsum": (c_int, [c_void_p] * 11 + [c_size_t] + [c_int] * 7 + [c_void_p]),
+    "dmvae_groupnorm_bwd_from_parts": (c_int, [c_void_p] * 5 + [c_size_t, c_int] + [c_void_p] * 6 + [c_size_t] + [c_int] * 5 + [c_void_p]),
+    "dmvae_groupnorm_bwd_from_parts_colsum": (c_int, [c_void_p] * 5 + [c_size_t, c_int] + [c_void_p] * 7 + [c_size_t] + [c_int] * 6 + [c_void_p]),
     "dmvae_groupnorm_bwd_reduce": (c_int, [c_void_p] * 9 + [c_size_t, c_int, c_int, c_int, c_int, c_int, c_int, c_void_p]),
     "dmvae_groupnorm_bwd_apply": (c_int, [c_void_p] * 8 + [c_int, c_int, c_int, c_int, c_int, c_float, c_void_p]),
     "dmvae_groupnorm_short_supported": (c_int, [c_int] * 5),
diff --git a/dmvae_amd/csrc/common.h b/dmvae_amd/csrc/common.h
--- a/dmvae_amd/csrc/common.h
+++ b/dmvae_amd/csrc/common.h
@@ -61,6 +61,10 @@
 }
 __device__ __forceinline__ float bf2f(bf16 v) { return (float)v; }
 __device__ __forceinline__ float sigmoidf_(float x) { return __builtin_amdgcn_rcpf(1.0f + __expf(-x)); }
+__device__ __forceinline__ float dswishf_(float t) {
+  const float sg = sigmoidf_(t);
+  return sg * (1.f + t * (1.f - sg));
+}
 __device__ __forceinline__ float sigmoid_exact(float x) { return 1.0f / (1.0f + expf(-x)); }
 
 __device__ __forceinline__ float dmvae_gelu_f(float x) {
diff --git a/dmvae_amd/csrc/conv_pp.hip b/dmvae_amd/csrc/conv_pp.hip
--- a/dmvae_amd/csrc/conv_pp.hip
+++ b/dmvae_amd/csrc/conv_pp.hip
@@ -21,6 +21,11 @@
   int Ml;
   unsigned wsRow, wsTap, wsChunk;
   float* gnpart;
+  const float* gn_stats;
+  const float* gn_gamma;
+  const float* gn_beta;
+  float* gnbpart;
+  int gn_groups, gn_cpg;
   unsigned* sched;
   unsigned long long* dbg;
 };
@@ -35,9 +40,10 @@
 }
 
 template <int TM, int TP, int WM, int WP, int NBUF, bool UPS, bool OUT_F32, bool KO, bool GEN = false, bool SUB = false, bool DYN = false, bool STATS = false,
-          bool HALO = false>
-__global__ __launch_bounds__(512) void conv_pp_kernel(Args a) {
+          bool HALO = false, bool GNB = false>
+__device__ __forceinline__ void conv_pp_body(const Args& a) {
 #if __HIP_DEVICE_COMPILE__
+  static_assert(!GNB || (HALO && !OUT_F32 && !STATS && !DYN), "GNB: the direct epilogue of the halo tiles");
   constexpr int BM = TM / WM / 32, BP = TP / WP / 32;
   constexpr int TILE_A = TM * 64, TILE_B = TP * 64, SLOT = TILE_A + TILE_B;
   constexpr int NPA = TM >= 128 ? TM / 128 : 1, NPB = TP / 128;
@@ -453,6 +459,29 @@
       it = (nK + 3) & ~3;
       it_ky = it_ch = 0;
     }
+    float gmu[GNB ? NQD : 1], grs[GNB ? NQD : 1], gga[GNB ? CL : 1], gbe[GNB ? CL : 1], gsa[GNB ? CL : 1], gsb[GNB ? CL : 1];
+    if constexpr (GNB) {
+      const __amdgpu_buffer_rsrc_t rSt = dmvae_buffer_rsrc(a.gn_stats, (unsigned)a.N * (unsigned)a.gn_groups * 8u);
+      const __amdgpu_buffer_rsrc_t rGa = dmvae_buffer_rsrc(a.gn_gamma, (unsigned)a.Cout * 4u), rBe = dmvae_buffer_rsrc(a.gn_beta, (unsigned)a.Cout * 4u);
+      int img, pin;
+      divmod_small(m0c, hw, inv_hw, small_m, img, pin);
+      const float inv_cpg = 1.0f / (float)a.gn_cpg;
+      const unsigned vo = c_ok ? (unsigned)col * 4u : SENT;
+#pragma unroll
+      for (int h = 0; h < NQD; h++) {
+        int gi, gr;
+        divmod_small(col + 4 * h, a.gn_cpg, inv_cpg, true, gi, gr);
+        const u32x2 s2 = __builtin_amdgcn_raw_buffer_load_b64(rSt, c_ok ? (unsigned)(img * a.gn_groups + gi) * 8u : SENT, 0, 0);
+        gmu[GNB ? h : 0] = __uint_as_float(s2[0]); grs[GNB ? h : 0] = __uint_as_float(s2[1]);
+        const u32x4 g4 = __builtin_amdgcn_raw_buffer_load_b128(rGa, vo == SENT ? SENT : vo + 16u * h, 0, 0);
+        const u32x4 b4 = __builtin_amdgcn_raw_buffer_load_b128(rBe, vo == SENT ? SENT : vo + 16u * h, 0, 0);
+#pragma unroll
+        for (int e = 0; e < 4; e++) {
+          gga[GNB ? 4 * h + e : 0] = __uint_as_float(g4[e]); gbe[GNB ? 4 * h + e : 0] = __uint_as_float(b4[e]);
+          gsa[GNB ? 4 * h + e : 0] = 0.f; gsb[GNB ? 4 * h + e : 0] = 0.f;
+        }
+      }
+    }
     issue_h(K0_{});
     stamp(work, 7);
     float s1[STATS ? NQD : 1], s2[STATS ? NQD : 1];
@@ -485,21 +514,23 @@
           for (int i = 0; i < CL; i++) {
             float x;
             asm volatile("v_accvgpr_read_b32 %0, %1" : "=v"(x) : "a"(acc[i][j][r]));
-            v[i] = x + bsv[i];
+            v[i] = x + (GNB ? 0.f : bsv[i]);
           }
           const int act = ACTC >= 0 ? ACTC : a.act;
+          float rf[RES ? CL : 1];
           if constexpr (RES) {
-            float rf[CL];
             {
               const rvec rv = rnx[RES ? r : 0];
 #pragma unroll
               for (int h = 0; h < CL / 2; h++) {
                 const unsigned wd = rv[h];
                 const bf16x2 b2 = *reinterpret_cast<const bf16x2*>(&wd);
-                rf[2 * h] = (float)b2[0]; rf[2 * h + 1] = (float)b2[1];
+                rf[RES ? 2 * h : 0] = (float)b2[0]; rf[RES ? 2 * h + 1 : 0] = (float)b2[1];
               }
             }
             if (j + 1 < BP16) fetch(j + 1, r);
+            if constexpr (GNB) {
+            } else
             if (act == 3) {
 #pragma unroll
               for (int e = 0; e < CL; e++) v[e] = rf[e] > 0.f ? v[e] : 0.f;
@@ -530,6 +561,17 @@
               s1[STATS ? h >> 1 : 0] = __builtin_amdgcn_fdot2_f32_bf16(p2, one2, s1[STATS ? h >> 1 : 0], false);
               s2[STATS ? h >> 1 : 0] = __builtin_amdgcn_fdot2_f32_bf16(p2, p2, s2[STATS ? h >> 1 : 0], false);
             }
+          }
+          if constexpr (GNB && RES) {
+#pragma unroll
+            for (int e = 0; e < CL; e++) {
+              const float d = __uint_as_float((e & 1) ? (pk[e >> 1] & 0xffff0000u) : (pk[e >> 1] << 16));
+              const float xh = (rf[RES ? e : 0] - gmu[GNB ? e >> 2 : 0]) * grs[GNB ? e >> 2 : 0];
+              const float g = d * dswishf_(xh * gga[GNB ? e : 0] + gbe[GNB ? e : 0]);
+              gsa[GNB ? e : 0] += g; gsb[GNB ? e : 0] += g * xh;
+            }
+#pragma unroll
+            for (int e = 0; e < CL; e++) asm volatile("" : "+v"(gsa[GNB ? e : 0]), "+v"(gsb[GNB ? e : 0]));
           }
           if constexpr (CL == 8) {
             const u32x4 o = {pk[0], pk[1], pk[2], pk[3]};
@@ -544,6 +586,21 @@
       }
     };
     using T_ = std::true_type; using F_ = std::false_type;
+    if constexpr (GNB) {
+      body(T_{}, std::integral_constant<int, 0>{});
+      const __amdgpu_buffer_rsrc_t rP = dmvae_buffer_rsrc(a.gnbpart, (unsigned)(a.M / TP) * (unsigned)WP * (unsigned)a.Cout * 8u);
+      const unsigned trow = (unsigned)(m0c / TP) * (unsigned)WP + (unsigned)wp;
+      const unsigned po = (gq == 0 && c_ok) ? (trow * (unsigned)a.Cout + (unsigned)col) * 8u : SENT;
+#pragma unroll
+      for (int h = 0; h < CL / 2; h++) {
+        float t[4] = {gsa[GNB ? 2 * h : 0], gsb[GNB ? 2 * h : 0], gsa[GNB ? 2 * h + 1 : 0], gsb[GNB ? 2 * h + 1 : 0]};
+#pragma unroll
+        for (int k = 0; k < 4; k++) { t[k] += __shfl_xor(t[k], 16, 64); t[k] += __shfl_xor(t[k], 32, 64); }
+        const u32x4 o = {__float_as_uint(t[0]), __float_as_uint(t[1]), __float_as_uint(t[2]), __float_as_uint(t[3])};
+        __builtin_amdgcn_raw_buffer_store_b128(o, rP, po == SENT ? SENT : po + 16u * h, 0, 0);
+        asm volatile("s_nop 0" :: "v"(o));
+      }
+    } else
     if (a.res) {
       if (a.act == 0) body(T_{}, std::integral_constant<int, 0>{});
       else if (a.act == 3) body(T_{}, std::integral_constant<int, 3>{});
@@ -767,6 +824,16 @@
     }
   }
 #endif
+}
+
+template <int TM, int TP, int WM, int WP, int NBUF, bool UPS, bool OUT_F32, bool KO, bool GEN = false, bool SUB = false, bool DYN = false, bool STATS = false,
+          bool HALO = false>
+__global__ __launch_bounds__(512) void conv_pp_kernel(Args a) {
+  conv_pp_body<TM, TP, WM, WP, NBUF, UPS, OUT_F32, KO, GEN, SUB, DYN, STATS, HALO, false>(a);
+}
+template <int TM, int TP>
+__global__ __launch_bounds__(512) void conv_pp_gnb_kernel(Args a) {
+  conv_pp_body<TM, TP, 2, 4, 4, false, false, true, false, false, false, false, true, true>(a);
 }
 
 constexpr int SCHED_WORDS = 16 + 512, SCHED_SLOTS = 32;
@@ -949,6 +1016,7 @@
   a.Ho = ho; a.Wo = wo; a.so = so; a.pd = pd; a.sd = sd;
   a.ks = d->ks; a.act = d->act; a.M = (int)M; a.ctiles = 0; a.dbg = g_dbg;
   a.Ml = d->n * d->h * d->w;
+  a.gn_stats = a.gn_gamma = a.gn_beta = nullptr; a.gnbpart = nullptr; a.gn_groups = a.gn_cpg = 0;
   a.gnpart = nullptr;
   if (gnpart && gn_tp && !d->out_f32 && (plain || sub) && !ups && gn_groups > 0 && d->cout % gn_groups == 0 && (d->cout / gn_groups) % 4 == 0) {
     const int tp = d->cout <= 128 ? 512 : 256;
@@ -969,3 +1037,61 @@
   if (ups) return f32 ? pick<true, true>(a, stream, false) : pick<true, false>(a, stream, false);
   return f32 ? pick<false, true>(a, stream, !plain) : pick<false, false>(a, stream, !plain);
 }
+
+namespace dmvae_conv_pp {
+template <int TM, int TP>
+int launch_gnb(Args a, hipStream_t st) {
+  a.ctiles = (a.Cout + TM - 1) / TM;
+  a.total = (a.M / TP) * a.ctiles;
+  const unsigned grid = a.total > 256 ? 256u : (unsigned)a.total;
+  constexpr int cwh = (TM / 2 / 32 >= 4) ? TM / 2 / 2 : TM / 2;
+  constexpr int group = 2 * TM * 64 + (TP + 16) * 64, epi_h = 8 * 32 * (cwh * 4 + 16);
+  constexpr int lds = group + (group > epi_h ? group : epi_h) + 1024;
+  DMVAE_LDS_OPTIN(lds, conv_pp_gnb_kernel<TM, TP>);
+  hipLaunchKernelGGL((conv_pp_gnb_kernel<TM, TP>), dim3(grid), dim3(512), lds, st, a);
+  DMVAE_CHECK_LAUNCH();
+  return 0;
+}
+
+static int gnb_tile(const dmvae_conv_desc* d, int groups) {
+  if (!d || groups <= 0 || !dmvae_conv_halo_applies(d)) return 0;
+  if (d->cout <= 64 || d->act != 0 || d->cout % groups != 0 || (d->cout / groups) % 4 != 0) return 0;
+  if (dynamic_on()) return 0;
+  const int tp = d->cout <= 128 ? 512 : 256, tm = d->cout <= 128 ? 128 : 256;
+  if (((long long)d->h * d->w) % tp != 0) return 0;
+  if (((long long)d->n * d->h * d->w / tp) * ((d->cout + tm - 1) / tm) < 256) return 0;
+  return tp;
+}
+}
+
+extern "C" int dmvae_conv2d_nhwc_gnbwd_supported(const dmvae_conv_desc* d, int groups) { return dmvae_conv_pp::gnb_tile(d, groups) ? 1 : 0; }
+
+extern "C" size_t dmvae_conv2d_nhwc_gnbwd_workspace(const dmvae_conv_desc* d, int groups) {
+  const int tp = dmvae_conv_pp::gnb_tile(d, groups);
+  if (!tp) return 0;
+  return (size_t)d->n * ((size_t)d->h * d->w / tp) * 4 * (size_t)d->cout * 2 * sizeof(float);
+}
+
+extern "C" int dmvae_conv2d_nhwc_gnbwd(const void* dy, const void* w, const void* gn_x, const void* stats, const void* gamma, const void* beta,
+                                       void* da, void* parts, size_t parts_bytes, int groups, const dmvae_conv_desc* d, hipStream_t stream) {
+  using namespace dmvae_conv_pp;
+  DMVAE_CHECK_ARG(dy && w && gn_x && stats && gamma && beta && da && parts && d, "conv2d_nhwc_gnbwd: null pointer");
+  const int tp = gnb_tile(d, groups);
+  DMVAE_CHECK_ARG(tp != 0, "conv2d_nhwc_gnbwd: unsupported shape (dmvae_conv2d_nhwc_gnbwd_supported is 0): n=%d h=%d w=%d cin=%d cout=%d groups=%d", d->n, d->h, d->w,
+                  d->cin, d->cout, groups);
+  DMVAE_CHECK_ARG(parts_bytes >= dmvae_conv2d_nhwc_gnbwd_workspace(d, groups), "conv2d_nhwc_gnbwd: partials buffer too small");
+  DMVAE_CHECK_ARG(d->w_layout == 0 || d->w_layout == 1, "conv2d_nhwc_gnbwd: w_layout %d (0 = tap-major, 1 = K-tile-major)", d->w_layout);
+  Args a;
+  a.wsRow = d->w_layout ? 64u : (unsigned)(9 * d->cin) * 2u;
+  a.wsTap = d->w_layout ? (unsigned)d->cout * 64u : (unsigned)d->cin * 2u;
+  a.wsChunk = d->w_layout ? 9u * (unsigned)d->cout * 64u : 64u;
+  a.x = (const bf16*)dy; a.w = (const bf16*)w; a.bias = nullptr; a.res = (const bf16*)gn_x; a.y = da;
+  a.N = d->n; a.Hi = d->h; a.Wi = d->w; a.Cin = d->cin; a.Cout = d->cout;
+  a.Ho = d->h; a.Wo = d->w; a.so = 1; a.pd = 1; a.sd = 1;
+  a.ks = 3; a.act = 0; a.M = d->n * d->h * d->w; a.ctiles = 0; a.total = 0; a.dbg = g_dbg;
+  a.Ml = a.M;
+  a.gnpart = nullptr; a.sched = nullptr;
+  a.gn_stats = (const float*)stats; a.gn_gamma = (const float*)gamma; a.gn_beta = (const float*)beta; a.gnbpart = (float*)parts;
+  a.gn_groups = groups; a.gn_cpg = d->cout / groups;
+  return tp == 512 ? launch_gnb<128, 512>(a, stream) : launch_gnb<256, 256>(a, stream);
+}
diff --git a/dmvae_amd/csrc/groupnorm.hip b/dmvae_amd/csrc/groupnorm.hip
--- a/dmvae_amd/csrc/groupnorm.hip
+++ b/dmvae_amd/csrc/groupnorm.hip
@@ -194,9 +194,7 @@
         const float xh = (v[e] - mu[e]) * rs[e];
         float dy = d[e];
         if (ACT == 1) {
-          const float t = xh * ga[e] + be[e];
-          const float sg = sigmoidf_(t);
-          dy *= sg * (1.f + t * (1.f - sg));
+          dy *= dswishf_(xh * ga[e] + be[e]);
         } else if (ACT == 2) {
           dy = xh * ga[e] + be[e] > 0.f ? dy : 0.2f * dy;
         }
@@ -214,8 +212,8 @@
   block_reduce_store(A, B, part, g, lane_c, prow, active);
 }
 
-__global__ void bwd_final_kernel(const float* __restrict__ part, const float* __restrict__ gamma, float* __restrict__ AB,
-                                 float* __restrict__ S, Geom g, int N) {
+__device__ __forceinline__ void bwd_final_body(const float* __restrict__ part, const float* __restrict__ gamma, float* __restrict__ AB,
+                                               float* __restrict__ S, const Geom& g, int N) {
   const int wid = (blockIdx.x * blockDim.x + threadIdx.x) >> 6, lane = threadIdx.x & 63;
   if (wid >= N * g.G) return;
   const int n = wid / g.G, grp = wid % g.G;
@@ -261,6 +259,14 @@
     __builtin_amdgcn_wave_barrier();
   }
   if (lane == 0) { S[wid * 2] = (float)s1; S[wid * 2 + 1] = (float)s2; }
+}
+__global__ void bwd_final_kernel(const float* __restrict__ part, const float* __restrict__ gamma, float* __restrict__ AB,
+                                 float* __restrict__ S, Geom g, int N) {
+  bwd_final_body(part, gamma, AB, S, g, N);
+}
+__global__ void bwd_from_parts_kernel(const float* __restrict__ part, const float* __restrict__ gamma, float* __restrict__ AB,
+                                      float* __restrict__ S, Geom g, int N) {
+  bwd_final_body(part, gamma, AB, S, g, N);
 }
 
 __global__ void bwd_param_kernel(const float* __restrict__ AB, float* __restrict__ dgamma, float* __restrict__ dbeta, int N, int C,
@@ -580,14 +586,16 @@
 }
 
 static int bwd_reduce_impl(const void* da, const void* x, const void* stats, const void* gamma, const void* beta, void* sums, void* dgamma, void* dbeta,
-                           void* workspace, size_t workspace_bytes, int n, int hw, int c, int groups, int act, int accumulate, bool with_param, hipStream_t stream);
+                           void* workspace, size_t workspace_bytes, int n, int hw, int c, int groups, int act, int accumulate, bool with_param, hipStream_t stream,
+                           const float* parts, int parts_chunks);
 extern "C" int dmvae_groupnorm_bwd_reduce(const void* da, const void* x, const void* stats, const void* gamma, const void* beta,
                                           void* sums, void* dgamma, void* dbeta, void* workspace, size_t workspace_bytes, int n, int hw,
                                           int c, int groups, int act, int accumulate, hipStream_t stream) {
-  return bwd_reduce_impl(da, x, stats, gamma, beta, sums, dgamma, dbeta, workspace, workspace_bytes, n, hw, c, groups, act, accumulate, true, stream);
+  return bwd_reduce_impl(da, x, stats, gamma, beta, sums, dgamma, dbeta, workspace, workspace_bytes, n, hw, c, groups, act, accumulate, true, stream, nullptr, 0);
 }
 static int bwd_reduce_impl(const void* da, const void* x, const void* stats, const void* gamma, const void* beta, void* sums, void* dgamma, void* dbeta,
-                           void* workspace, size_t workspace_bytes, int n, int hw, int c, int groups, int act, int accumulate, bool with_param, hipStream_t stream) {
+                           void* workspace, size_t workspace_bytes, int n, int hw, int c, int groups, int act, int accumulate, bool with_param, hipStream_t stream,
+                           const float* parts, int parts_chunks) {
   Geom g;
   DMVAE_CHECK_ARG(da && x && stats && gamma && beta && sums && workspace, "groupnorm_bwd_reduce: null pointer");
   DMVAE_CHECK_ARG(act >= 0 && act <= 2, "groupnorm_bwd_reduce: act must be 0, 1 or 2");
@@ -595,6 +603,14 @@
   DMVAE_CHECK_ARG(workspace_bytes >= dmvae_groupnorm_workspace(n, hw, c, groups), "groupnorm_bwd_reduce: workspace too small");
   float* part = (float*)workspace;
   float* AB = part + (size_t)n * g.nchunk * c * 2;
+  if (parts) {
+    DMVAE_CHECK_ARG(act == 1 && parts_chunks > 0, "groupnorm_bwd_from_parts: swish only, parts_chunks > 0");
+    Geom gp = g;
+    gp.nchunk = parts_chunks;
+    hipLaunchKernelGGL(bwd_from_parts_kernel, dim3((n * groups + 3) / 4), dim3(256), 0, stream, parts, (const float*)gamma, AB, (float*)sums, gp, n);
+    DMVAE_CHECK_LAUNCH();
+    return 0;
+  }
   const dim3 grid(g.nchunk, n);
 #define DMVAE_GN_PART(A) hipLaunchKernelGGL(bwd_partial_kernel<A>, grid, dim3(256), 0, stream, (const bf16*)da, (const bf16*)x, \
                                             (const float*)stats, (const float*)gamma, (const float*)beta, part, g)
@@ -617,7 +633,7 @@
   DMVAE_CHECK_ARG(make_geom(g, n, hw, c, groups) == 0, "groupnorm_bwd_reduce: unsupported shape n=%d hw=%d c=%d groups=%d", n, hw, c, groups);
   *AB = (float*)workspace + (size_t)n * g.nchunk * c * 2;
   *S = *AB + (size_t)n * c * 2;
-  return bwd_reduce_impl(da, x, stats, gamma, beta, *S, nullptr, nullptr, workspace, workspace_bytes, n, hw, c, groups, act, 0, false, stream);
+  return bwd_reduce_impl(da, x, stats, gamma, beta, *S, nullptr, nullptr, workspace, workspace_bytes, n, hw, c, groups, act, 0, false, stream, nullptr, 0);
 }
 
 extern "C" int dmvae_groupnorm_bwd_apply(const void* da, const void* x, const void* dres, const void* stats, const void* sums,
@@ -636,9 +652,9 @@
   return 0;
 }
 
-extern "C" int dmvae_groupnorm_bwd(const void* da, const void* x, const void* dres, const void* stats, const void* gamma,
-                                   const void* beta, void* dx, void* dgamma, void* dbeta, void* workspace, size_t workspace_bytes,
-                                   int n, int hw, int c, int groups, int act, int accumulate, hipStream_t stream) {
+static int bwd_impl(const void* da, const void* x, const void* dres, const void* stats, const void* gamma,
+                    const void* beta, void* dx, void* dgamma, void* dbeta, void* workspace, size_t workspace_bytes,
+                    int n, int hw, int c, int groups, int act, int accumulate, hipStream_t stream, const float* parts, int parts_chunks) {
   Geom g;
   DMVAE_CHECK_ARG(da && x && stats && gamma && beta && dx && workspace, "groupnorm_bwd: null pointer");
   DMVAE_CHECK_ARG(act >= 0 && act <= 2, "groupnorm_bwd: act must be 0, 1 or 2");
@@ -646,7 +662,7 @@
   DMVAE_CHECK_ARG(workspace_bytes >= dmvae_groupnorm_workspace(n, hw, c, groups), "groupnorm_bwd: workspace too small");
   float* AB = (float*)workspace + (size_t)n * g.nchunk * c * 2;
   float* S = AB + (size_t)n * c * 2;
-  int rc = bwd_reduce_impl(da, x, stats, gamma, beta, S, dgamma, dbeta, workspace, workspace_bytes, n, hw, c, groups, act, accumulate, false, stream);
+  int rc = bwd_reduce_impl(da, x, stats, gamma, beta, S, dgamma, dbeta, workspace, workspace_bytes, n, hw, c, groups, act, accumulate, false, stream, parts, parts_chunks);
   if (rc) return rc;
   const bool par = dgamma && dbeta;
   const dim3 grid(g.nchunk, n);
@@ -661,9 +677,9 @@
 
 int dmvae_colsum_final(const float* part, float* out, int nparts, int C, int accumulate, hipStream_t stream);
 
-extern "C" int dmvae_groupnorm_bwd_colsum(const void* da, const void* x, const void* dres, const void* stats, const void* gamma, const void* beta, void* dx,
-                                          void* dgamma, void* dbeta, void* colsum, void* workspace, size_t workspace_bytes, int n, int hw, int c, int groups,
-                                          int act, int accumulate, int colsum_accumulate, hipStream_t stream) {
+static int bwd_colsum_impl(const void* da, const void* x, const void* dres, const void* stats, const void* gamma, const void* beta, void* dx,
+                           void* dgamma, void* dbeta, void* colsum, void* workspace, size_t workspace_bytes, int n, int hw, int c, int groups,
+                           int act, int accumulate, int colsum_accumulate, hipStream_t stream, const float* parts, int parts_chunks) {
   Geom g;
   DMVAE_CHECK_ARG(da && x && stats && gamma && beta && dx && colsum && workspace, "groupnorm_bwd_colsum: null pointer");
   DMVAE_CHECK_ARG(act >= 0 && act <= 2, "groupnorm_bwd_colsum: act must be 0, 1 or 2");
@@ -671,7 +687,7 @@
   DMVAE_CHECK_ARG(workspace_bytes >= dmvae_groupnorm_workspace(n, hw, c, groups), "groupnorm_bwd_colsum: workspace too small");
   float* AB = (float*)workspace + (size_t)n * g.nchunk * c * 2;
   float* S = AB + (size_t)n * c * 2;
-  int rc = bwd_reduce_impl(da, x, stats, gamma, beta, S, dgamma, dbeta, workspace, workspace_bytes, n, hw, c, groups, act, accumulate, false, stream);
+  int rc = bwd_reduce_impl(da, x, stats, gamma, beta, S, dgamma, dbeta, workspace, workspace_bytes, n, hw, c, groups, act, accumulate, false, stream, parts, parts_chunks);
   if (rc) return rc;
   const bool par = dgamma && dbeta;
   float* colpart = (float*)workspace;
@@ -683,6 +699,40 @@
 #undef DMVAE_GN_BAPPLYC
   DMVAE_CHECK_LAUNCH();
   return dmvae_colsum_final(colpart, (float*)colsum, n * g.nchunk, c, colsum_accumulate, stream);
+}
+
+extern "C" int dmvae_groupnorm_bwd(const void* da, const void* x, const void* dres, const void* stats, const void* gamma,
+                                   const void* beta, void* dx, void* dgamma, void* dbeta, void* workspace, size_t workspace_bytes,
+                                   int n, int hw, int c, int groups, int act, int accumulate, hipStream_t stream) {
+  return bwd_impl(da, x, dres, stats, gamma, beta, dx, dgamma, dbeta, workspace, workspace_bytes, n, hw, c, groups, act, accumulate, stream, nullptr, 0);
+}
+extern "C" int dmvae_groupnorm_bwd_colsum(const void* da, const void* x, const void* dres, const void* stats, const void* gamma, const void* beta, void* dx,
+                                          void* dgamma, void* dbeta, void* colsum, void* workspace, size_t workspace_bytes, int n, int hw, int c, int groups,
+                                          int act, int accumulate, int colsum_accumulate, hipStream_t stream) {
+  return bwd_colsum_impl(da, x, dres, stats, gamma, beta, dx, dgamma, dbeta, colsum, workspace, workspace_bytes, n, hw, c, groups, act, accumulate, colsum_accumulate,
+                         stream, nullptr, 0);
+}
+
+static int parts_chunks_of(const void* parts, size_t parts_bytes, int n, int hw, int c, int tp) {
+  if (!parts || n <= 0 || c <= 0 || (tp != 256 && tp != 512) || hw <= 0 || hw % tp != 0) return 0;
+  const int chunks = hw / tp * 4;
+  return parts_bytes >= (size_t)n * chunks * c * 2 * sizeof(float) ? chunks : 0;
+}
+extern "C" int dmvae_groupnorm_bwd_from_parts(const void* da, const void* x, const void* dres, const void* stats, const void* parts, size_t parts_bytes, int tp,
+                                              const void* gamma, const void* beta, void* dx, void* dgamma, void* dbeta, void* workspace, size_t workspace_bytes,
+                                              int n, int hw, int c, int groups, int accumulate, hipStream_t stream) {
+  const int chunks = parts_chunks_of(parts, parts_bytes, n, hw, c, tp);
+  DMVAE_CHECK_ARG(chunks > 0, "groupnorm_bwd_from_parts: partials of n=%d hw=%d c=%d at pixel tile %d: bad shape or buffer too small", n, hw, c, tp);
+  return bwd_impl(da, x, dres, stats, gamma, beta, dx, dgamma, dbeta, workspace, workspace_bytes, n, hw, c, groups, 1, accumulate, stream, (const float*)parts, chunks);
+}
+extern "C" int dmvae_groupnorm_bwd_from_parts_colsum(const void* da, const void* x, const void* dres, const void* stats, const void* parts, size_t parts_bytes, int tp,
+                                                     const void* gamma, const void* beta, void* dx, void* dgamma, void* dbeta, void* colsum, void* workspace,
+                                                     size_t workspace_bytes, int n, int hw, int c, int groups, int accumulate, int colsum_accumulate,
+                                                     hipStream_t stream) {
+  const int chunks = parts_chunks_of(parts, parts_bytes, n, hw, c, tp);
+  DMVAE_CHECK_ARG(chunks > 0, "groupnorm_bwd_from_parts_colsum: partials of n=%d hw=%d c=%d at pixel tile %d: bad shape or buffer too small", n, hw, c, tp);
+  return bwd_colsum_impl(da, x, dres, stats, gamma, beta, dx, dgamma, dbeta, colsum, workspace, workspace_bytes, n, hw, c, groups, 1, accumulate, colsum_accumulate,
+                         stream, (const float*)parts, chunks);
 }
 
 static int convout_geom(Geom& g, int n, int h, int w, int c, int groups) {
diff --git a/dmvae_amd/functional.py b/dmvae_amd/functional.py
--- a/dmvae_amd/functional.py
+++ b/dmvae_amd/functional.py
@@ -170,6 +170,16 @@
     return sw.shape[1] == c and ops.groupnorm_short_supported(n, x.numel() // (n * c), c, sw.shape[0])
 
 
+GN_BWD_FROM_CONV = True
+
+
+def _dgrad_gn_bwd(dy, w_dgrad, x, st, gw, gb, **kw):
+    if GN_BWD_FROM_CONV and x.dtype == bf16 and ops.conv2d_nhwc_gnbwd_supported(dy, w_dgrad):
+        da, parts = ops.conv2d_nhwc_gnbwd(dy, w_dgrad, x, st, gw, gb, ks=3)
+        return ops.groupnorm_bwd_from_parts(da, x, st, parts, gw, gb, **kw)
+    return ops.groupnorm_bwd(ops.conv2d_nhwc(dy, w_dgrad, ks=3), x, st, gw, gb, True, **kw)
+
+
 class ResnetBlockFn(torch.autograd.Function):
 
     @staticmethod
@@ -195,10 +205,10 @@
         dy = _c(dy)
         c1b, c2b, sb = ctx.bias_params
         dc2w, dc2b = ops.conv2d_nhwc_wgrad(dy, a2, 3, dw_out=_dst(c2w), db_out=_dst(c2b))
-        da2 = ops.conv2d_nhwc(dy, packed(c2w, True), ks=3)
-        dh1, dn2w, dn2b = ops.groupnorm_bwd(da2, h1, st2, n2w, n2b, True, dg_out=_dst(n2w), db_out=_dst(n2b))
+        dh1, dn2w, dn2b = _dgrad_gn_bwd(dy, packed(c2w, True), h1, st2, n2w, n2b, dg_out=_dst(n2w), db_out=_dst(n2b))
         dc1w, dc1b = ops.conv2d_nhwc_wgrad(dh1, a1, 3, dw_out=_dst(c1w), db_out=_dst(c1b))
-        da1 = ops.conv2d_nhwc(dh1, packed(c1w, True), ks=3)
+        if sw is not None and ctx.short:
+            da1 = ops.conv2d_nhwc(dh1, packed(c1w, True), ks=3)
         if sw is None:
             dxs, dsw, dsb = dy, None, None
         else:
@@ -208,7 +218,7 @@
                                                          want_colsum=ctx.want_colsum)
                 return dx, dn1w, dn1b, dc1w, dc1b, dn2w, dn2b, dc2w, dc2b, dsw, dsb
             dxs = ops.conv2d_nhwc(dy, packed(sw, True), ks=1)
-        dx, dn1w, dn1b = ops.groupnorm_bwd(da1, x, st1, n1w, n1b, True, dres=dxs, dg_out=_dst(n1w), db_out=_dst(n1b), want_colsum=ctx.want_colsum)
+        dx, dn1w, dn1b = _dgrad_gn_bwd(dh1, packed(c1w, True), x, st1, n1w, n1b, dres=dxs, dg_out=_dst(n1w), db_out=_dst(n1b), want_colsum=ctx.want_colsum)
         return dx, dn1w, dn1b, dc1w, dc1b, dn2w, dn2b, dc2w, dc2b, dsw, dsb
 
 
diff --git a/dmvae_amd/ops.py b/dmvae_amd/ops.py
--- a/dmvae_amd/ops.py
+++ b/dmvae_amd/ops.py
@@ -549,6 +549,76 @@
         return dx, dg, db
     check(L.dmvae_groupnorm_bwd(da.data_ptr(), x.data_ptr(), _ptr(dres), stats.data_ptr(), gamma.data_ptr(), beta.data_ptr(), dx.data_ptr(),
                                 _ptr(dg), _ptr(db), ws.data_ptr(), ws.numel(), n, hw, c, groups, int(swish), 0, _stream()), "groupnorm_bwd")
+    return dx, dg, db
+
+
+def conv2d_nhwc_gnbwd_supported(dy: torch.Tensor, w_packed: torch.Tensor, groups: int = 32, ks: int = 3) -> bool:
+    if parity.on() or dy.dtype != bf16 or w_packed.dtype != bf16 or ks != 3 or dy.dim() != 4:
+        return False
+    n, h, w_, cin = dy.shape
+    d = ConvDesc(n, h, w_, cin, w_packed.shape[0], 3, 0, ACT_NONE, 0, 1, 0)
+    return bool(_lib.lib().dmvae_conv2d_nhwc_gnbwd_supported(ctypes.byref(d), groups))
+
+
+def conv2d_nhwc_gnbwd(dy: torch.Tensor, w_packed: torch.Tensor, gn_x: torch.Tensor, stats: torch.Tensor, gamma: torch.Tensor, beta: torch.Tensor, ks: int = 3,
+                      groups: int = 32):
+    if not conv2d_nhwc_gnbwd_supported(dy, w_packed, groups, ks):
+        return conv2d_nhwc(dy, w_packed, ks=ks), None
+    dy = _req(dy, bf16, "dy")
+    gn_x = _req(gn_x, bf16, "gn_x")
+    w_packed = _req(w_packed, bf16, "w_packed")
+    _req(stats, f32, "stats"); _req(gamma, f32, "gamma"); _req(beta, f32, "beta")
+    n, h, w_, cin = dy.shape
+    cout = w_packed.shape[0]
+    assert w_packed.shape[1] == 9 and w_packed.shape[2] == cin, (w_packed.shape, cin)
+    assert tuple(gn_x.shape) == (n, h, w_, cout) and tuple(stats.shape) == (n, groups, 2) and gamma.numel() == cout and beta.numel() == cout
+    d = ConvDesc(n, h, w_, cin, cout, 3, 0, ACT_NONE, 0, 1, 0)
+    L = _lib.lib()
+    nbytes = L.dmvae_conv2d_nhwc_gnbwd_workspace(ctypes.byref(d), groups)
+    tp = 512 if cout <= 128 else 256
+    parts = torch.empty(n, h * w_ // tp, 4, cout, 2, dtype=f32, device=dy.device)
+    assert parts.numel() * 4 == nbytes, (parts.shape, nbytes)
+    da = torch.empty(n, h, w_, cout, dtype=bf16, device=dy.device)
+    timing = KERNEL_TIMING
+    if timing is not None:
+        e0 = torch.cuda.Event(enable_timing=True)
+        e0.record()
+    check(L.dmvae_conv2d_nhwc_gnbwd(dy.data_ptr(), _weight_operand(w_packed, d), gn_x.data_ptr(), stats.data_ptr(), gamma.data_ptr(), beta.data_ptr(),
+                                    da.data_ptr(), parts.data_ptr(), parts.numel() * 4, groups, ctypes.byref(d), _stream()), "conv2d_nhwc_gnbwd")
+    if timing is not None:
+        e1 = torch.cuda.Event(enable_timing=True)
+        e1.record()
+        timing.append(("conv_pp_gnb_kernel<%s>" % ("128, 512" if cout <= 128 else "256, 256"), e0, e1, 2.0 * n * h * w_ * cout * cin * 9))
+    return da, parts
+
+
+def groupnorm_bwd_from_parts(da: torch.Tensor, x: torch.Tensor, stats: torch.Tensor, parts: torch.Tensor, gamma: torch.Tensor, beta: torch.Tensor,
+                             dres: Optional[torch.Tensor] = None, groups: int = 32, dg_out: Optional[torch.Tensor] = None,
+                             db_out: Optional[torch.Tensor] = None, want_colsum: bool = False):
+    da = _req(da, bf16, "da")
+    x = _req(x, bf16, "x")
+    parts = _req(parts, f32, "parts")
+    n, c = x.shape[0], x.shape[-1]
+    hw = x.numel() // (n * c)
+    tp = 512 if c <= 128 else 256
+    assert tuple(parts.shape) == (n, hw // tp, 4, c, 2), (parts.shape, x.shape)
+    L = _lib.lib()
+    ws = workspace(L.dmvae_groupnorm_workspace(n, hw, c, groups), x.device)
+    dx = torch.empty_like(x)
+    dg = dg_out if dg_out is not None else torch.empty(c, dtype=f32, device=x.device)
+    db = db_out if db_out is not None else torch.empty(c, dtype=f32, device=x.device)
+    if dres is not None:
+        _req(dres, bf16, "dres")
+    if want_colsum:
+        cs = torch.empty(c, dtype=f32, device=x.device)
+        check(L.dmvae_groupnorm_bwd_from_parts_colsum(da.data_ptr(), x.data_ptr(), _ptr(dres), stats.data_ptr(), parts.data_ptr(), parts.numel() * 4, tp,
+                                                      gamma.data_ptr(), beta.data_ptr(), dx.data_ptr(), dg.data_ptr(), db.data_ptr(), cs.data_ptr(), ws.data_ptr(),
+                                                      ws.numel(), n, hw, c, groups, 0, 0, _stream()), "groupnorm_bwd_from_parts_colsum")
+        dx._dmvae_colsum = (cs, dx._version, dx.data_ptr())
+        return dx, dg, db
+    check(L.dmvae_groupnorm_bwd_from_parts(da.data_ptr(), x.data_ptr(), _ptr(dres), stats.data_ptr(), parts.data_ptr(), parts.numel() * 4, tp, gamma.data_ptr(),
+                                           beta.data_ptr(), dx.data_ptr(), dg.data_ptr(), db.data_ptr(), ws.data_ptr(), ws.numel(), n, hw, c, groups, 0, _stream()),
+          "groupnorm_bwd_from_parts")
     return dx, dg, db
 
 
diff --git a/include/dmvae_hip.h b/include/dmvae_hip.h
--- a/include/dmvae_hip.h
+++ b/include/dmvae_hip.h
@@ -36,6 +36,11 @@
 int dmvae_conv2d_nhwc_fwd_gnstats(const void* x, const void* w, const void* bias, const void* residual, void* y, void* stats, void* workspace,
                                   size_t workspace_bytes, int groups, float eps, const dmvae_conv_desc* d, dmvae_stream_t stream);
 
+int dmvae_conv2d_nhwc_gnbwd_supported(const dmvae_conv_desc* d, int groups);
+size_t dmvae_conv2d_nhwc_gnbwd_workspace(const dmvae_conv_desc* d, int groups);
+int dmvae_conv2d_nhwc_gnbwd(const void* dy, const void* w, const void* gn_x, const void* stats, const void* gamma, const void* beta,
+                            void* da, void* parts, size_t parts_bytes, int groups, const dmvae_conv_desc* d, dmvae_stream_t stream);
+
 size_t dmvae_conv2d_nhwc_wgrad_workspace(const dmvae_conv_desc* d);
 int dmvae_conv2d_nhwc_wgrad(const void* dy, const void* a, void* dw, void* dbias, void* workspace,
                             size_t workspace_bytes, const dmvae_conv_desc* d, int accumulate,
@@ -61,6 +66,13 @@
 int dmvae_groupnorm_bwd_colsum(const void* da, const void* x, const void* dres, const void* stats, const void* gamma, const void* beta, void* dx,
                                void* dgamma, void* dbeta, void* colsum, void* workspace, size_t workspace_bytes, int n, int hw, int c, int groups, int act,
                                int accumulate, int colsum_accumulate, dmvae_stream_t stream);
+int dmvae_groupnorm_bwd_from_parts(const void* da, const void* x, const void* dres, const void* stats, const void* parts, size_t parts_bytes, int tp,
+                                   const void* gamma, const void* beta, void* dx, void* dgamma, void* dbeta, void* workspace, size_t workspace_bytes,
+                                   int n, int hw, int c, int groups, int accumulate, dmvae_stream_t stream);
+int dmvae_groupnorm_bwd_from_parts_colsum(const void* da, const void* x, const void* dres, const void* stats, const void* parts, size_t parts_bytes, int tp,
+                                          const void* gamma, const void* beta, void* dx, void* dgamma, void* dbeta, void* colsum, void* workspace,
+                                          size_t workspace_bytes, int n, int hw, int c, int groups, int accumulate, int colsum_accumulate,
+                                          dmvae_stream_t stream);
 int dmvae_groupnorm_bwd_reduce(const void* da, const void* x, const void* stats, const void* gamma, const void* beta,
                                void* sums, void* dgamma, void* dbeta, void* workspace, size_t workspace_bytes, int n,
                                int hw, int c, int groups, int act, int accumulate, dmvae_stream_t stream);
```

Measured after the change: 497.1, median of 6. About the same (+0.9%).
